# thygate/stable-diffusion-webui-depthmap-script

Hardware: AMD Instinct MI355X
Metric: depth+stereo pairs/sec @1024x1024 (higher is better)
Workload: dtype f16 (network) / f64 (stereo, normal map); 1 GPU; BASELINE config c3: MiDaS 3.1 DPT BEiT-L/16 512 forward (fp16, random-init weights seed 0, net 512x512, 1025 tokens) + depth->u16 + create_stereoimages(polylines_sharp, left-right, divergence 2.5%) + create_normalmap (Sobel 3) on 32 x 1024x1024 RGB per GPU, inputs resident in HBM; depth_network=dpt_beit_large_512, height=1024, width=1024, forward_launch=eager, library_convolutions=MIOpen, heuristic solver choice, overlap=single stream, parallelism=units sharded over 1 GPU(s), no data-path collective

## Files before the change

include/depthstereo.h:

```cpp
#ifndef DEPTHSTEREO_H
#define DEPTHSTEREO_H

#include <stddef.h>
#include <stdint.h>

#ifdef __cplusplus
extern "C" {
#endif

#define DS_VERSION 100

#define DS_OK            0
#define DS_EINVAL       -1
#define DS_EUNSUPPORTED -2
#define DS_EHIP         -3
#define DS_ENOMEM       -4

#define DS_DEPTH_U16 0
#define DS_DEPTH_F32 1
#define DS_DEPTH_F64 2

#define DS_FILL_NONE                0
#define DS_FILL_NAIVE               1
#define DS_FILL_NAIVE_INTERPOLATING 2
#define DS_FILL_POLYLINES_SOFT      3
#define DS_FILL_POLYLINES_SHARP     4

typedef struct ds_ctx ds_ctx;

int ds_version(void);
const char *ds_last_error(void);
int ds_ctx_create(ds_ctx **out, int device);
int ds_ctx_destroy(ds_ctx *ctx);

typedef struct ds_eye {
    double divergence_px;
    double separation_px;
    uint8_t *out;
    int64_t out_row_stride;
    int64_t out_img_stride;
} ds_eye;

int ds_stereo_warp(ds_ctx *ctx, const uint8_t *image, const void *depth, int depth_dtype,
                   int n, int h, int w, int c, double exponent, const double *pow_lut,
                   int fill, const ds_eye *eyes, int n_eyes, void *stream);

int ds_depth_minmax(ds_ctx *ctx, const void *depth, int depth_dtype, int n, int h, int w,
                    double *minmax_out, void *stream);

int ds_profile_enable(ds_ctx *ctx, int enable);
int ds_profile_last_ms(ds_ctx *ctx, float *render_ms, float *exact_ms);

#define DS_KT_LINEAR_GELU      0
#define DS_KT_ATTENTION        1
#define DS_KT_LINEAR_RESIDUAL  2
#define DS_KT_LINEAR           3
#define DS_KT_LINEAR_VT        4
#define DS_KT_CONV3X3          5
#define DS_KT_LINEAR_READOUT   6
#define DS_KT_LINEAR_SHUFFLE   7
#define DS_KT_NORMALMAP        8
#define DS_KT_RAGGED          12
int ds_kernel_timer_enable(ds_ctx *ctx, int enable);
int ds_kernel_timer_read(ds_ctx *ctx, int kind, int64_t *launches, double *total_ms);
int ds_kernel_timer_read_each(ds_ctx *ctx, int kind, float *ms_out, int64_t capacity, int64_t *launches);

int ds_stereo_last_exact_rows(ds_ctx *ctx, int64_t *rows_out, void *stream);
int ds_stereo_last_stats(ds_ctx *ctx, int64_t *stats_out, void *stream);

int ds_copy_view(ds_ctx *ctx, const uint8_t *src, int64_t src_row_stride, int64_t src_img_stride,
                 uint8_t *dst, int64_t dst_row_stride, int64_t dst_img_stride,
                 int n, int h, int64_t row_bytes, void *stream);

int ds_overlap_red_cyan(ds_ctx *ctx, const uint8_t *im1, int64_t im1_row_stride, int64_t im1_img_stride,
                        const uint8_t *im2, int64_t im2_row_stride, int64_t im2_img_stride,
                        int n, int h, int w, int c, uint8_t *out, void *stream);

int ds_normalmap(ds_ctx *ctx, const uint16_t *depth, int n, int h, int w, int pre_blur,
                 int sobel_ksize, int post_blur, int invert, uint8_t *out, void *stream);

int ds_normalmap_f64(ds_ctx *ctx, const double *depth, int n, int h, int w, int pre_blur,
                     int sobel_ksize, int post_blur, int invert, uint8_t *out, void *stream);

int ds_normalmap_gradient_f32(ds_ctx *ctx, const float *depth, int n, int h, int w, int invert, uint8_t *out, void *stream);

int ds_normalmap_gradient_f16(ds_ctx *ctx, const void *depth, int n, int h, int w, int invert, uint8_t *out, void *stream);

int ds_normalmap_gradient_blur_f32(ds_ctx *ctx, const float *depth, int n, int h, int w, int pre_blur, int post_blur, int invert,
                                   uint8_t *out, void *stream);

int ds_normalmap_wrap(ds_ctx *ctx, const uint16_t *depth, int n, int h, int w, int pre_blur,
                      int sobel_ksize, int post_blur, int invert, uint8_t *out, void *stream);
int ds_normalmap_f64_wrap(ds_ctx *ctx, const double *depth, int n, int h, int w, int pre_blur,
                          int sobel_ksize, int post_blur, int invert, uint8_t *out, void *stream);
int ds_normalmap_gradient_f32_wrap(ds_ctx *ctx, const float *depth, int n, int h, int w, int invert, uint8_t *out, void *stream);
int ds_normalmap_gradient_f16_wrap(ds_ctx *ctx, const void *depth, int n, int h, int w, int invert, uint8_t *out, void *stream);
int ds_normalmap_gradient_blur_f32_wrap(ds_ctx *ctx, const float *depth, int n, int h, int w, int pre_blur, int post_blur, int invert,
                                        uint8_t *out, void *stream);

int ds_bilateral_u16(ds_ctx *ctx, const uint16_t *depth, int n, int h, int w, int radius, const double *ws, const double *wr,
                     int wrap, double *out, void *stream);

int ds_normalmap_selfcheck(ds_ctx *ctx, unsigned long long k0, unsigned long long stride, unsigned long long count,
                           unsigned long long *mismatches, void *stream);

int ds_depth_to_u16(ds_ctx *ctx, const float *pred, int n, int h, int w, int invert,
                    uint16_t *out, float *norm_out, void *stream);

int ds_colorize_u16(ds_ctx *ctx, const uint16_t *depth, int n, int h, int w, const double *vmin_vmax,
                    const uint8_t *lut_rgba, int lut_n, uint8_t *out, void *stream);

int ds_convert_to_i16(ds_ctx *ctx, const void *arr, int is_f64, int64_t count, uint16_t *out, void *stream);

#define DS_PIX_U8  0
#define DS_PIX_U16 1
#define DS_PIX_I32 2
#define DS_PIX_F32 3

int ds_resize_lanczos(ds_ctx *ctx, const void *src, int pix, int n, int in_h, int in_w, int64_t src_px_stride, int64_t src_row_stride,
                      int64_t src_img_stride, void *dst, int out_h, int out_w, const int32_t *h_bounds, const void *h_coeffs, int h_taps,
                      const int32_t *v_bounds, const void *v_coeffs, int v_taps, void *tmp, void *stream);

#define DS_CD_WIDEN       0
#define DS_CD_SINGLE_BAND 1
#define DS_CD_MULTI_BAND  2
#define DS_CD_WORKSPACE_BLOCKS 256
int ds_custom_depth_to_f64(ds_ctx *ctx, const void *src, int pix, int n, int h, int w, int64_t src_px_stride, int64_t src_row_stride,
                           int64_t src_img_stride, int rule, double *out, double *workspace, void *stream);

#define DS_DTYPE_F16  1
#define DS_DTYPE_BF16 2
#define DS_DTYPE_F32  3

int ds_attention_fwd(ds_ctx *ctx, const void *qk, const void *vt, const void *bias_packed, void *out,
                     int B, int Np, int H, int n_valid, float scale, int dtype, void *stream);

int ds_attention_bias_pack(ds_ctx *ctx, const float *bias, int H, int n, int Np, int dtype, void *packed, void *stream);

int ds_attention_reload_env(void);

int ds_preprocess_bicubic(ds_ctx *ctx, const void *images, void *out, int batch, int in_h, int in_w, int out_h, int out_w,
                          int flip_channels, const float *mean, const float *std, int dtype, void *stream);

int ds_residual_layernorm(ds_ctx *ctx, const void *x, const void *branch, const void *gamma, const void *ln_weight,
                          const void *ln_bias, void *x_out, void *h_out, int64_t rows, int channels, float eps, int dtype,
                          void *stream);

int ds_reassemble_readout(ds_ctx *ctx, const void *proj, const void *clsvec, void *out, int batch, int tokens, int channels,
                          int dtype, void *stream);

int ds_bias_act_nhwc(ds_ctx *ctx, const void *x, const void *bias, const void *res1, const void *res2, void *out,
                     int64_t elements, int channels, int relu, int dtype, void *stream);

int ds_group_norm_nchw(ds_ctx *ctx, const void *x, const void *gamma, const void *beta, const void *res, void *out, int n, int channels,
                       int hw, int groups, float eps, int relu, int dtype, void *stream);

int ds_linear(ds_ctx *ctx, const void *x, const void *w, const void *bias, void *y, int64_t rows, int64_t out_features,
              int64_t in_features, int64_t ldy, int act, int dtype, void *stream);

int ds_linear_residual(ds_ctx *ctx, const void *x, const void *w, const void *bias, const void *gamma, const void *res, void *y,
                       int64_t rows, int64_t out_features, int64_t in_features, int dtype, void *stream);

int ds_linear_vt(ds_ctx *ctx, const void *w_v, const void *h, void *vt, int64_t channels, int64_t batch, int64_t tokens,
                 int64_t in_features, int dtype, void *stream);

int ds_linear_qkv(ds_ctx *ctx, const void *h, const void *w_qk, const void *b_qk, const void *w_v, void *qk, void *vt,
                  int64_t batch, int64_t tokens, int64_t qk_features, int64_t v_channels, int64_t in_features, int dtype, void *stream);

int ds_linear_shuffle(ds_ctx *ctx, const void *x, const void *w, const void *bias, void *y, int64_t pixels, int64_t in_features,
                      int width, int stride, int out_channels, int dtype, void *stream);

int ds_linear_readout(ds_ctx *ctx, const void *x, const void *w_tok, const void *cls_vec, void *y, int64_t images,
                      int64_t tokens_padded, int64_t tokens, int64_t out_features, int64_t in_features, int dtype, void *stream);

int ds_row_stats(ds_ctx *ctx, const void *x, void *stats, int64_t rows, int channels, float eps, int dtype, void *stream);
int ds_linear_ln(ds_ctx *ctx, const void *x, const void *w_scaled, const float *colsum, const void *bias, const void *stats, void *y,
                 int64_t rows, int64_t out_features, int64_t in_features, int64_t ldy, int act, int dtype, void *stream);
int ds_linear_vt_ln(ds_ctx *ctx, const void *w_v_scaled, const float *colsum, const void *x, const void *stats, void *vt,
                    int64_t channels, int64_t batch, int64_t tokens, int64_t in_features, int dtype, void *stream);

int ds_linear_reload_env(void);

int ds_conv3x3_nhwc(ds_ctx *ctx, const void *x, const void *w, const void *bias, const void *res1, const void *res2, void *y,
                    int batch, int height, int width, int in_channels, int out_channels, int act, int dtype, void *stream);

int ds_conv3x3_nhwc_circular(ds_ctx *ctx, const void *x, const void *w, const void *bias, const void *res1, const void *res2, void *y,
                             int batch, int height, int width, int in_channels, int out_channels, int act, int dtype, void *stream);

int ds_upsample_bilinear_nhwc(ds_ctx *ctx, const void *in, void *out, int batch, int channels, int in_h, int in_w,
                              int out_h, int out_w, int align_corners, int dtype, void *stream);

int ds_dpt_head_tail(ds_ctx *ctx, const void *x, int batch, int in_h, int in_w, int out_h, int out_w,
                     const void *conv3_wfrag, const float *conv3_bias, const float *conv1_weight, float conv1_bias,
                     int relu_out, void *out, int dtype, void *stream);

int ds_dpt_head_tail_circular(ds_ctx *ctx, const void *x, int batch, int in_h, int in_w, int out_h, int out_w,
                              const void *conv3_wfrag, const float *conv3_bias, const float *conv1_weight, float conv1_bias,
                              int relu_out, void *out, int dtype, void *stream);

int ds_gconv3x3_nhwc_f32(ds_ctx *ctx, const float *x, const float *w_gtio, const float *bias, float *y, int batch, int height, int width,
                         int channels, int channels_per_group, int relu, void *stream);
int ds_add_relu_f32(ds_ctx *ctx, const float *a, const float *b, float *y, int64_t count, void *stream);

int ds_bias_act_f32(ds_ctx *ctx, const float *x, const float *bias, const float *res, float *y, int64_t pixels, int channels, int relu,
                    void *stream);

int ds_dwconv_nhwc(ds_ctx *ctx, const void *x, const float *w, const float *bias_in, const float *bias, void *y, int batch, int in_h,
                   int in_w, int channels, int out_h, int out_w, int kernel, int stride, int pad_top, int pad_left, int dtype, void *stream);
int ds_relu_cat_f32(ds_ctx *ctx, const float *a, const float *b, float *y, int batch, int64_t plane, int channels_a, int channels_b, int layout,
                    void *stream);

int ds_boost_blend(ds_ctx *ctx, float *dst, int64_t dst_row_stride, int height, int width, const void *patches,
                   int n_patches, const float *preds, int pred_size, const float *mask_template, int mask_size,
                   void *stream);

#ifdef __cplusplus
}
#endif
#endif
```

stable-diffusion-webui-depthmap-script_amd/build_native.py:

```python
import os
import shutil
import subprocess
import sys

HERE = os.path.dirname(os.path.abspath(__file__))
CSRC = os.path.join(HERE, "csrc")
EXPERIMENTS = bool(os.environ.get("DS_EXPERIMENTS"))
OUT = os.path.join(HERE, "libdepthstereo_hip_experiments.so" if EXPERIMENTS else "libdepthstereo_hip.so")
OBJ_DIR = os.path.join(HERE, "build", "experiments") if EXPERIMENTS else os.path.join(HERE, "build")
SOURCES = ["ds_api.hip", "ds_stereo.hip", "ds_stereo_polylines.hip", "ds_normalmap.hip", "ds_attention.hip", "ds_attention4.hip", "ds_encoder_ops.hip", "ds_boost.hip", "ds_heatmap.hip", "ds_linear.hip", "ds_gconv.hip", "ds_dwconv.hip", "ds_resample.hip", "ds_bilateral.hip"]
FLAGS = ["--offload-arch=gfx950", "-O3", "-std=c++17", "-ffp-contract=off", "-fno-fast-math", "-fPIC",
         "-fvisibility=hidden", "-Wall", "-Wno-unused-function",
         "-mllvm", "-amdgpu-mfma-vgpr-form=1"]


if EXPERIMENTS:
    FLAGS.append("-DDS_EXPERIMENTS")


EXTRA_FLAGS = {"ds_attention4.hip": ["-fno-slp-vectorize"]}


def hipcc():
    for cand in (shutil.which("hipcc"), "/opt/rocm/bin/hipcc"):
        if cand and os.path.exists(cand):
            return cand
    raise RuntimeError("hipcc not found")


def needs_build():
    if not os.path.exists(OUT):
        return True
    t = os.path.getmtime(OUT)
    deps = [os.path.join(CSRC, f) for f in os.listdir(CSRC)] + [os.path.join(HERE, "..", "include", "depthstereo.h")]
    return any(os.path.getmtime(d) > t for d in deps)


def build(force=False, verbose=True):
    if not force and not needs_build():
        return OUT
    objs = []
    procs = []
    os.makedirs(OBJ_DIR, exist_ok=True)
    for s in SOURCES:
        o = os.path.join(OBJ_DIR, s.replace(".hip", ".o"))
        cmd = [hipcc()] + FLAGS + EXTRA_FLAGS.get(s, []) + ["-c", os.path.join(CSRC, s), "-o", o]
        if verbose:
            print(" ".join(cmd), flush=True)
        procs.append((s, subprocess.Popen(cmd)))
        objs.append(o)
    for s, p in procs:
        if p.wait() != 0:
            raise RuntimeError(f"hipcc failed on {s}")
    cmd = [hipcc(), "--offload-arch=gfx950", "-shared", "-fPIC", "-o", OUT] + objs
    if verbose:
        print(" ".join(cmd), flush=True)
    subprocess.check_call(cmd)
    return OUT


if __name__ == "__main__":
    build(force="--force" in sys.argv)
    print(OUT)
```

stable-diffusion-webui-depthmap-script_amd/csrc/ds_common.h:

```cpp
#pragma once
#include <hip/hip_runtime.h>
#include <stdint.h>
#include <stdio.h>
#include <string.h>

#include "../../include/depthstereo.h"

#define DS_API extern "C" __attribute__((visibility("default")))

void ds_set_error(const char *fmt, ...);

#define DS_HIP_CHECK(expr)                                                              \
    do {                                                                                \
        hipError_t _e = (expr);                                                         \
        if (_e != hipSuccess) {                                                         \
            ds_set_error("%s failed: %s (%s:%d)", #expr, hipGetErrorString(_e), __FILE__, __LINE__); \
            return DS_EHIP;                                                             \
        }                                                                               \
    } while (0)

#define DS_REQUIRE(cond, code, ...)      \
    do {                                 \
        if (!(cond)) {                   \
            ds_set_error(__VA_ARGS__);   \
            return (code);               \
        }                                \
    } while (0)

#define DS_KT_KINDS 24
#define DS_KT_RING 1024
struct ds_ctx {
    int device;
    void *minmax;      size_t minmax_bytes;
    void *partials;    size_t partials_bytes;
    void *row_flags;   size_t row_flags_bytes;
    void *row_list;    size_t row_list_bytes;
    void *exact_ws;    size_t exact_ws_bytes;
    void *tmp_a;       size_t tmp_a_bytes;
    void *tmp_b;       size_t tmp_b_bytes;
    void *zero_line;   size_t zero_line_bytes;
    int zero_line_cleared;
    void *lin_ws;      size_t lin_ws_bytes;
    void *lin_ws_cleared;
    void *gn_ws;       size_t gn_ws_bytes;
    int ncu;
    int64_t last_exact_rows_valid;
    int profile;
    hipEvent_t ev[4];
    int ev_created, ev_recorded;
    int ktimer;
    hipEvent_t (*kt_ev[DS_KT_KINDS])[2];
    int kt_n[DS_KT_KINDS];
};

int ds_kt_begin(ds_ctx *ctx, int kind, hipStream_t st);
void ds_kt_end(ds_ctx *ctx, int kind, int slot, hipStream_t st);

int ds_ctx_reserve(ds_ctx *ctx, void **slot, size_t *cur, size_t need);

__device__ __forceinline__ uint8_t ds_f64_to_u8(double v)
{
    if (!(v == v)) return 0;
    if (v >= 9.2e18 || v <= -9.2e18) return 0;
    return (uint8_t)(long long)v;
}

__device__ __forceinline__ int ds_reflect101(int i, int n)
{
    if (n == 1) return 0;
    while (i < 0 || i >= n) { if (i < 0) i = -i; else i = 2 * (n - 1) - i; }
    return i;
}
__device__ __forceinline__ int ds_mod(int i, int n)
{
    i %= n;
    return i < 0 ? i + n : i;
}
__device__ __forceinline__ int ds_wrap_prev(int i, int n) { return i > 0 ? i - 1 : n - 1; }
__device__ __forceinline__ int ds_wrap_next(int i, int n) { return i + 1 < n ? i + 1 : 0; }

__device__ __forceinline__ double ds_wave_min(double v)
{
    for (int o = 32; o > 0; o >>= 1) { double t = __shfl_xor(v, o, 64); v = t < v ? t : v; }
    return v;
}
__device__ __forceinline__ double ds_wave_max(double v)
{
    for (int o = 32; o > 0; o >>= 1) { double t = __shfl_xor(v, o, 64); v = t > v ? t : v; }
    return v;
}

template <int DT> struct ds_depth_traits;
template <> struct ds_depth_traits<DS_DEPTH_U16> {
    typedef uint16_t T;
    __device__ static __forceinline__ double norm(T v, double mn, double mx) {
        return (double)(uint16_t)(v - (uint16_t)mn) / (double)(uint16_t)((uint16_t)mx - (uint16_t)mn);
    }
};
template <> struct ds_depth_traits<DS_DEPTH_F32> {
    typedef float T;
    __device__ static __forceinline__ double norm(T v, double mn, double mx) {
        float den = (float)mx - (float)mn;
        float q = (v - (float)mn) / den;
        return (double)q;
    }
};
template <> struct ds_depth_traits<DS_DEPTH_F64> {
    typedef double T;
    __device__ static __forceinline__ double norm(T v, double mn, double mx) {
        return (v - mn) / (mx - mn);
    }
};
```

stable-diffusion-webui-depthmap-script_amd/csrc/ds_encoder_ops.hip:

```cpp
#include <stdlib.h>
#include <string.h>

#include <algorithm>

#include "ds_common.h"

template <int BF16> struct eo_traits;
template <> struct eo_traits<0> { typedef _Float16 T; };
template <> struct eo_traits<1> { typedef __bf16 T; };

template <int BF16, int EPL, int W>
__global__ __launch_bounds__(256) void k_residual_layernorm(const void *x_, const void *o_, const void *gamma_, const void *lnw_,
                                                             const void *lnb_, void *xout_, void *hout_, int M, float eps)
{
    typedef typename eo_traits<BF16>::T T;
    constexpr int C = EPL * 64;
    const int lane = threadIdx.x & 63;
    const int row = blockIdx.x * 4 + (threadIdx.x >> 6);
    if (row >= M) return;
    const T *x = (const T *)x_ + (size_t)row * C;
    const T *o = o_ ? (const T *)o_ + (size_t)row * C : nullptr;
    const T *gamma = (const T *)gamma_, *lnw = (const T *)lnw_, *lnb = (const T *)lnb_;
    T *xout = xout_ ? (T *)xout_ + (size_t)row * C : nullptr;
    T *hout = (T *)hout_ + (size_t)row * C;
    float v[EPL];
    float sum = 0.f;
#pragma unroll
    for (int k = 0; k < EPL / W; k++) {
        const int idx = (k * 64 + lane) * W;
        T xv[W], ov[W], gv[W];
        __builtin_memcpy(xv, x + idx, sizeof(xv));
        if (o) {
            __builtin_memcpy(ov, o + idx, sizeof(ov));
            if (gamma) __builtin_memcpy(gv, gamma + idx, sizeof(gv));
        }
        T rv[W];
#pragma unroll
        for (int t = 0; t < W; t++) {
            float f = (float)xv[t];
            if (o) f += (gamma ? (float)gv[t] : 1.0f) * (float)ov[t];
            rv[t] = (T)f;
            v[k * W + t] = (float)rv[t];
            sum += v[k * W + t];
        }
        if (o && xout) __builtin_memcpy(xout + idx, rv, sizeof(rv));
    }
#pragma unroll
    for (int s = 32; s > 0; s >>= 1) sum += __shfl_xor(sum, s, 64);
    const float mean = sum * (1.0f / C);
    float sq = 0.f;
#pragma unroll
    for (int i = 0; i < EPL; i++) { const float d = v[i] - mean; sq += d * d; }
#pragma unroll
    for (int s = 32; s > 0; s >>= 1) sq += __shfl_xor(sq, s, 64);
    const float rstd = rsqrtf(sq * (1.0f / C) + eps);
#pragma unroll
    for (int k = 0; k < EPL / W; k++) {
        const int idx = (k * 64 + lane) * W;
        T wv[W], bv[W], hv[W];
        __builtin_memcpy(wv, lnw + idx, sizeof(wv));
        __builtin_memcpy(bv, lnb + idx, sizeof(bv));
#pragma unroll
        for (int t = 0; t < W; t++) hv[t] = (T)((v[k * W + t] - mean) * rstd * (float)wv[t] + (float)bv[t]);
        __builtin_memcpy(hout + idx, hv, sizeof(hv));
    }
}

template <int BF16>
static int eo_launch(int C, const void *x, const void *o, const void *gamma, const void *lnw, const void *lnb, void *xout, void *hout,
                     int M, float eps, hipStream_t st)
{
    dim3 grid((M + 3) / 4), block(256);
    switch (C) {
    case 384: hipLaunchKernelGGL((k_residual_layernorm<BF16, 6, 2>), grid, block, 0, st, x, o, gamma, lnw, lnb, xout, hout, M, eps); break;
    case 768: hipLaunchKernelGGL((k_residual_layernorm<BF16, 12, 4>), grid, block, 0, st, x, o, gamma, lnw, lnb, xout, hout, M, eps); break;
    case 1024: hipLaunchKernelGGL((k_residual_layernorm<BF16, 16, 8>), grid, block, 0, st, x, o, gamma, lnw, lnb, xout, hout, M, eps); break;
    case 1536: hipLaunchKernelGGL((k_residual_layernorm<BF16, 24, 8>), grid, block, 0, st, x, o, gamma, lnw, lnb, xout, hout, M, eps); break;
    default: ds_set_error("ds_residual_layernorm: channel count %d not built (384, 768, 1024, 1536)", C); return DS_EUNSUPPORTED;
    }
    return DS_OK;
}

DS_API int ds_residual_layernorm(ds_ctx *ctx, const void *x, const void *branch, const void *gamma, const void *ln_weight,
                                 const void *ln_bias, void *x_out, void *h_out, int64_t rows, int channels, float eps, int dtype,
                                 void *stream)
{
    DS_REQUIRE(ctx && x && ln_weight && ln_bias && h_out, DS_EINVAL, "ds_residual_layernorm: null argument");
    DS_REQUIRE(rows > 0 && rows < (1ll << 31), DS_EINVAL, "ds_residual_layernorm: bad row count");
    DS_REQUIRE(dtype == DS_DTYPE_F16 || dtype == DS_DTYPE_BF16, DS_EINVAL, "ds_residual_layernorm: dtype must be f16 or bf16");
    DS_REQUIRE(branch == nullptr || x_out != nullptr, DS_EINVAL, "ds_residual_layernorm: x_out is required with a branch");
    DS_REQUIRE(((uintptr_t)x & 15) == 0 && ((uintptr_t)h_out & 15) == 0 && ((uintptr_t)branch & 15) == 0 && ((uintptr_t)x_out & 15) == 0,
               DS_EINVAL, "ds_residual_layernorm: operands must be 16-byte aligned");
    DS_HIP_CHECK(hipSetDevice(ctx->device));
    int rc = dtype == DS_DTYPE_F16
        ? eo_launch<0>(channels, x, branch, gamma, ln_weight, ln_bias, x_out, h_out, (int)rows, eps, (hipStream_t)stream)
        : eo_launch<1>(channels, x, branch, gamma, ln_weight, ln_bias, x_out, h_out, (int)rows, eps, (hipStream_t)stream);
    if (rc) return rc;
    DS_HIP_CHECK(hipGetLastError());
    return DS_OK;
}

template <int BF16, int EPL, int W>
__global__ __launch_bounds__(256) void k_row_stats(const void *x_, float2 *stats, int M, float eps)
{
    typedef typename eo_traits<BF16>::T T;
    constexpr int C = EPL * 64;
    const int lane = threadIdx.x & 63;
    const int row = blockIdx.x * 4 + (threadIdx.x >> 6);
    if (row >= M) return;
    const T *x = (const T *)x_ + (size_t)row * C;
    float v[EPL];
    float sum = 0.f;
#pragma unroll
    for (int k = 0; k < EPL / W; k++) {
        T xv[W];
        __builtin_memcpy(xv, x + (k * 64 + lane) * W, sizeof(xv));
#pragma unroll
        for (int t = 0; t < W; t++) { v[k * W + t] = (float)xv[t]; sum += v[k * W + t]; }
    }
#pragma unroll
    for (int s = 32; s > 0; s >>= 1) sum += __shfl_xor(sum, s, 64);
    const float mean = sum * (1.0f / C);
    float sq = 0.f;
#pragma unroll
    for (int i = 0; i < EPL; i++) { const float d = v[i] - mean; sq += d * d; }
#pragma unroll
    for (int s = 32; s > 0; s >>= 1) sq += __shfl_xor(sq, s, 64);
    const float rstd = rsqrtf(sq * (1.0f / C) + eps);
    if (lane == 0) stats[row] = make_float2(rstd, -mean * rstd);
}

DS_API int ds_row_stats(ds_ctx *ctx, const void *x, void *stats, int64_t rows, int channels, float eps, int dtype, void *stream)
{
    DS_REQUIRE(ctx && x && stats, DS_EINVAL, "ds_row_stats: null argument");
    DS_REQUIRE(rows > 0 && rows < (1ll << 31), DS_EINVAL, "ds_row_stats: bad row count");
    DS_REQUIRE(dtype == DS_DTYPE_F16 || dtype == DS_DTYPE_BF16, DS_EINVAL, "ds_row_stats: dtype must be f16 or bf16");
    DS_REQUIRE(((uintptr_t)x & 15) == 0 && ((uintptr_t)stats & 15) == 0, DS_EINVAL, "ds_row_stats: operands must be 16-byte aligned");
    DS_HIP_CHECK(hipSetDevice(ctx->device));
    dim3 grid((unsigned)((rows + 3) / 4)), block(256);
    hipStream_t st = (hipStream_t)stream;
    float2 *out = (float2 *)stats;
    const int M = (int)rows;
#define RS_CASE(C_, EPL_, W_) case C_: if (dtype == DS_DTYPE_F16) hipLaunchKernelGGL((k_row_stats<0, EPL_, W_>), grid, block, 0, st, x, out, M, eps); \
                                       else hipLaunchKernelGGL((k_row_stats<1, EPL_, W_>), grid, block, 0, st, x, out, M, eps); break;
    switch (channels) {
    RS_CASE(384, 6, 2) RS_CASE(768, 12, 4) RS_CASE(1024, 16, 8) RS_CASE(1536, 24, 8)
    default: ds_set_error("ds_row_stats: channel count %d not built (384, 768, 1024, 1536)", channels); return DS_EUNSUPPORTED;
    }
#undef RS_CASE
    DS_HIP_CHECK(hipGetLastError());
    return DS_OK;
}

template <int BF16>
__global__ __launch_bounds__(256) void k_upsample_bilinear_nhwc(const void *in_, void *out_, int C8, int ih, int iw, int oh, int ow,
                                                                 float sy, float sx, int align_corners)
{
    typedef typename eo_traits<BF16>::T T;
    const unsigned i = blockIdx.x * 256u + threadIdx.x;
    if (i >= (unsigned)ow * (unsigned)C8) return;
    const int ox = (int)(i / (unsigned)C8), c8 = (int)(i - (unsigned)ox * (unsigned)C8);
    const int b = blockIdx.z;
    float fx;
    if (align_corners) fx = sx * ox;
    else fx = fmaxf(sx * (ox + 0.5f) - 0.5f, 0.f);
    const int x0 = min((int)fx, iw - 1), x1 = min(x0 + 1, iw - 1);
    const float tx = fx - x0;
    const T *in = (const T *)in_ + (size_t)b * ih * iw * C8 * 8 + (size_t)c8 * 8;
    int py0 = -1, py1 = -1;
    T a[8], bq[8], c[8], d[8], o[8];
#pragma unroll
    for (int r = 0; r < 2; r++) {
        const int oy = 2 * (int)blockIdx.y + r;
        if (oy >= oh) break;
        float fy;
        if (align_corners) fy = sy * oy;
        else fy = fmaxf(sy * (oy + 0.5f) - 0.5f, 0.f);
        const int y0 = min((int)fy, ih - 1), y1 = min(y0 + 1, ih - 1);
        const float ty = fy - y0;
        if (y0 == py1 && y0 != py0) {
#pragma unroll
            for (int k = 0; k < 8; k++) { a[k] = c[k]; bq[k] = d[k]; }
        } else if (y0 != py0) {
            __builtin_memcpy(a, in + ((size_t)y0 * iw + x0) * C8 * 8, 16);
            __builtin_memcpy(bq, in + ((size_t)y0 * iw + x1) * C8 * 8, 16);
        }
        if (y1 != py1 || r == 0) {
            if (y1 == y0) {
#pragma unroll
                for (int k = 0; k < 8; k++) { c[k] = a[k]; d[k] = bq[k]; }
            } else {
                __builtin_memcpy(c, in + ((size_t)y1 * iw + x0) * C8 * 8, 16);
                __builtin_memcpy(d, in + ((size_t)y1 * iw + x1) * C8 * 8, 16);
            }
        }
        py0 = y0; py1 = y1;
        const float w00 = (1.f - ty) * (1.f - tx), w01 = (1.f - ty) * tx, w10 = ty * (1.f - tx), w11 = ty * tx;
#pragma unroll
        for (int k = 0; k < 8; k++)
            o[k] = (T)(w00 * (float)a[k] + w01 * (float)bq[k] + w10 * (float)c[k] + w11 * (float)d[k]);
        __builtin_memcpy((T *)out_ + ((((size_t)b * oh + oy) * ow) * C8 + i) * 8, o, 16);
    }
}

DS_API int ds_upsample_bilinear_nhwc(ds_ctx *ctx, const void *in, void *out, int batch, int channels, int in_h, int in_w,
                                     int out_h, int out_w, int align_corners, int dtype, void *stream)
{
    DS_REQUIRE(ctx && in && out, DS_EINVAL, "ds_upsample_bilinear_nhwc: null argument");
    DS_REQUIRE(batch > 0 && channels > 0 && (channels % 8) == 0 && in_h > 0 && in_w > 0 && out_h > 0 && out_w > 0, DS_EINVAL,
               "ds_upsample_bilinear_nhwc: bad shape (channels must be a multiple of 8)");
    DS_REQUIRE(dtype == DS_DTYPE_F16 || dtype == DS_DTYPE_BF16, DS_EINVAL, "ds_upsample_bilinear_nhwc: dtype must be f16 or bf16");
    DS_REQUIRE(((uintptr_t)in & 15) == 0 && ((uintptr_t)out & 15) == 0, DS_EINVAL, "ds_upsample_bilinear_nhwc: 16-byte alignment");
    DS_HIP_CHECK(hipSetDevice(ctx->device));
    float sy, sx;
    if (align_corners) {
        sy = out_h > 1 ? (float)(in_h - 1) / (float)(out_h - 1) : 0.f;
        sx = out_w > 1 ? (float)(in_w - 1) / (float)(out_w - 1) : 0.f;
    } else {
        sy = (float)in_h / (float)out_h;
        sx = (float)in_w / (float)out_w;
    }
    const int C8 = channels / 8;
    DS_REQUIRE((long long)out_w * C8 < (1ll << 31) && out_h <= 65535 && batch <= 65535, DS_EUNSUPPORTED, "ds_upsample_bilinear_nhwc: tensor too large");
    dim3 grid((unsigned)(((long long)out_w * C8 + 255) / 256), (unsigned)((out_h + 1) / 2), (unsigned)batch);
    if (dtype == DS_DTYPE_F16)
        hipLaunchKernelGGL((k_upsample_bilinear_nhwc<0>), grid, dim3(256), 0, (hipStream_t)stream, in, out, C8, in_h, in_w, out_h, out_w, sy, sx, align_corners);
    else
        hipLaunchKernelGGL((k_upsample_bilinear_nhwc<1>), grid, dim3(256), 0, (hipStream_t)stream, in, out, C8, in_h, in_w, out_h, out_w, sy, sx, align_corners);
    DS_HIP_CHECK(hipGetLastError());
    return DS_OK;
}

struct PreParams {
    const uint8_t *in;
    void *out;
    int B, ih, iw, oh, ow, flip;
    float sy, sx;
    float mean[3], istd[3];
    long long total;
};

__device__ __forceinline__ void pre_cubic(float t, float *c)
{
    const float A = -0.75f;
    const float x0 = t + 1.0f, x3 = 2.0f - t, x2 = 1.0f - t;
    c[0] = ((A * x0 - 5.0f * A) * x0 + 8.0f * A) * x0 - 4.0f * A;
    c[1] = ((A + 2.0f) * t - (A + 3.0f)) * t * t + 1.0f;
    c[2] = ((A + 2.0f) * x2 - (A + 3.0f)) * x2 * x2 + 1.0f;
    c[3] = ((A * x3 - 5.0f * A) * x3 + 8.0f * A) * x3 - 4.0f * A;
}

template <int DT>
__global__ __launch_bounds__(256) void k_preprocess_bicubic(PreParams P)
{
    const long long idx = (long long)blockIdx.x * 256 + threadIdx.x;
    if (idx >= P.total) return;
    const int ox = (int)(idx % P.ow);
    long long r = idx / P.ow;
    const int oy = (int)(r % P.oh);
    const int b = (int)(r / P.oh);
    const float fy = P.sy * ((float)oy + 0.5f) - 0.5f, fx = P.sx * ((float)ox + 0.5f) - 0.5f;
    const float fy0 = floorf(fy), fx0 = floorf(fx);
    float cy[4], cx[4];
    pre_cubic(fy - fy0, cy);
    pre_cubic(fx - fx0, cx);
    const int iy = (int)fy0, ix = (int)fx0;
    const uint8_t *img = P.in + (size_t)b * P.ih * P.iw * 3;
    float acc[3] = {0.f, 0.f, 0.f};
#pragma unroll
    for (int ky = 0; ky < 4; ky++) {
        const int y = min(max(iy - 1 + ky, 0), P.ih - 1);
        const uint8_t *row = img + (size_t)y * P.iw * 3;
        float h[3] = {0.f, 0.f, 0.f};
#pragma unroll
        for (int kx = 0; kx < 4; kx++) {
            const int x = min(max(ix - 1 + kx, 0), P.iw - 1);
            const uint8_t *px = row + (size_t)x * 3;
#pragma unroll
            for (int c = 0; c < 3; c++) h[c] += cx[kx] * ((float)px[c] / 255.0f);
        }
#pragma unroll
        for (int c = 0; c < 3; c++) acc[c] += cy[ky] * h[c];
    }
    float o[3];
#pragma unroll
    for (int c = 0; c < 3; c++) o[c] = (acc[P.flip ? 2 - c : c] - P.mean[c]) * P.istd[c];
    if (DT == 2) {
        float *q = (float *)P.out + (size_t)idx * 3;
        q[0] = o[0]; q[1] = o[1]; q[2] = o[2];
    } else {
        typedef typename eo_traits<DT == 1 ? 1 : 0>::T T;
        T *q = (T *)P.out + (size_t)idx * 3;
        q[0] = (T)o[0]; q[1] = (T)o[1]; q[2] = (T)o[2];
    }
}

DS_API int ds_preprocess_bicubic(ds_ctx *ctx, const void *images, void *out, int batch, int in_h, int in_w, int out_h, int out_w,
                                 int flip_channels, const float *mean, const float *std, int dtype, void *stream)
{
    DS_REQUIRE(ctx && images && out && mean && std, DS_EINVAL, "ds_preprocess_bicubic: null argument");
    DS_REQUIRE(batch > 0 && in_h > 0 && in_w > 0 && out_h > 0 && out_w > 0, DS_EINVAL, "ds_preprocess_bicubic: bad shape");
    DS_REQUIRE(dtype == DS_DTYPE_F16 || dtype == DS_DTYPE_BF16 || dtype == DS_DTYPE_F32, DS_EINVAL, "ds_preprocess_bicubic: dtype must be f16, bf16 or f32");
    DS_REQUIRE(std[0] != 0.f && std[1] != 0.f && std[2] != 0.f, DS_EINVAL, "ds_preprocess_bicubic: std must be non-zero");
    DS_HIP_CHECK(hipSetDevice(ctx->device));
    PreParams P;
    P.in = (const uint8_t *)images; P.out = out;
    P.B = batch; P.ih = in_h; P.iw = in_w; P.oh = out_h; P.ow = out_w; P.flip = flip_channels ? 1 : 0;
    P.sy = (float)in_h / (float)out_h; P.sx = (float)in_w / (float)out_w;
    for (int c = 0; c < 3; c++) { P.mean[c] = mean[c]; P.istd[c] = 1.0f / std[c]; }
    P.total = (long long)batch * out_h * out_w;
    DS_REQUIRE((P.total + 255) / 256 < (1ll << 31), DS_EUNSUPPORTED, "ds_preprocess_bicubic: tensor too large");
    dim3 grid((unsigned)((P.total + 255) / 256));
    hipStream_t st = (hipStream_t)stream;
    if (dtype == DS_DTYPE_F16) hipLaunchKernelGGL((k_preprocess_bicubic<0>), grid, dim3(256), 0, st, P);
    else if (dtype == DS_DTYPE_BF16) hipLaunchKernelGGL((k_preprocess_bicubic<1>), grid, dim3(256), 0, st, P);
    else hipLaunchKernelGGL((k_preprocess_bicubic<2>), grid, dim3(256), 0, st, P);
    DS_HIP_CHECK(hipGetLastError());
    return DS_OK;
}

#define HT_TW 32
#define HT_PW (HT_TW + 2)

typedef _Float16 ht_f16x8 __attribute__((ext_vector_type(8)));
typedef __bf16 ht_bf16x8 __attribute__((ext_vector_type(8)));
typedef float ht_f32x16 __attribute__((ext_vector_type(16)));

struct HeadTailParams {
    const void *x;
    const void *wfrag;
    const float *b2, *w3;
    void *out;
    float b3;
    int B, ih, iw, oh, ow, relu_out;
    float sy, sx;
};

template <int BF16, int RPW, int CIRC = 0>
__global__ __launch_bounds__(256) void k_dpt_head_tail(HeadTailParams P)
{
    typedef typename eo_traits<BF16>::T T;
    constexpr int HT_TH = 4 * RPW;
    constexpr int HT_NPIX = (HT_TH + 2) * HT_PW;
    extern __shared__ __attribute__((aligned(16))) unsigned char s_act[];
    const int tid = threadIdx.x, wave = tid >> 6, lane = tid & 63, hi = lane >> 5, l31 = lane & 31;
    const int b = blockIdx.z, ty0 = blockIdx.y * HT_TH, tx0 = blockIdx.x * HT_TW;
    const T *x = (const T *)P.x + (size_t)b * P.ih * P.iw * 128;

    for (int i0 = tid; i0 < HT_NPIX * 16; i0 += 256 * 4) {
        T a[4][8], bq[4][8], cq[4][8], d[4][8];
        float w00[4], w01[4], w10[4], w11[4];
        bool inside[4], live[4];
#pragma unroll
        for (int u = 0; u < 4; u++) {
            const int i = i0 + u * 256;
            live[u] = i < HT_NPIX * 16;
            const int pix = min(i, HT_NPIX * 16 - 1) >> 4, chunk = i & 15;
            const int r = pix / HT_PW, c = pix - r * HT_PW;
            int oy = ty0 - 1 + r, ox = tx0 - 1 + c;
            if constexpr (CIRC) {
                oy = oy < 0 ? oy + P.oh : (oy >= P.oh ? oy - P.oh : oy);
                ox = ox < 0 ? ox + P.ow : (ox >= P.ow ? ox - P.ow : ox);
                oy = min(oy, P.oh - 1); ox = min(ox, P.ow - 1);
                inside[u] = live[u];
            } else {
                inside[u] = live[u] && oy >= 0 && oy < P.oh && ox >= 0 && ox < P.ow;
            }
            const float fy = P.sy * max(oy, 0), fx = P.sx * max(ox, 0);
            const int y0 = min((int)fy, P.ih - 1), x0 = min((int)fx, P.iw - 1);
            const int y1 = min(y0 + 1, P.ih - 1), x1 = min(x0 + 1, P.iw - 1);
            const float ty = fy - y0, tx = fx - x0;
            w00[u] = (1.f - ty) * (1.f - tx); w01[u] = (1.f - ty) * tx; w10[u] = ty * (1.f - tx); w11[u] = ty * tx;
            __builtin_memcpy(a[u], x + ((size_t)y0 * P.iw + x0) * 128 + chunk * 8, 16);
            __builtin_memcpy(bq[u], x + ((size_t)y0 * P.iw + x1) * 128 + chunk * 8, 16);
            __builtin_memcpy(cq[u], x + ((size_t)y1 * P.iw + x0) * 128 + chunk * 8, 16);
            __builtin_memcpy(d[u], x + ((size_t)y1 * P.iw + x1) * 128 + chunk * 8, 16);
        }
#pragma unroll
        for (int u = 0; u < 4; u++) {
            if (!live[u]) continue;
            const int i = i0 + u * 256;
            const int pix = i >> 4, chunk = i & 15;
            T o[8];
#pragma unroll
            for (int k = 0; k < 8; k++)
                o[k] = inside[u] ? (T)(w00[u] * (float)a[u][k] + w01[u] * (float)bq[u][k] + w10[u] * (float)cq[u][k] + w11[u] * (float)d[u][k])
                                 : (T)0.f;
            __builtin_memcpy(s_act + pix * 256 + ((chunk ^ (pix & 15)) << 4), o, 16);
        }
    }
    __syncthreads();

    ht_f32x16 acc[RPW];
#pragma unroll
    for (int rr = 0; rr < RPW; rr++)
#pragma unroll
        for (int r = 0; r < 16; r++) acc[rr][r] = 0.f;
    const T *wf = (const T *)P.wfrag + ((size_t)hi * 32 + l31) * 8;
#pragma unroll
    for (int tap = 0; tap < 9; tap++) {
        const int dy = tap / 3, dx = tap - dy * 3;
#pragma unroll
        for (int s = 0; s < 8; s++) {
            uint4 wraw = *reinterpret_cast<const uint4 *>(wf + (size_t)(tap * 8 + s) * 2 * 32 * 8);
#pragma unroll
            for (int rr = 0; rr < RPW; rr++) {
                const int pix = (RPW * wave + rr + dy) * HT_PW + l31 + dx;
                const uint4 araw = *reinterpret_cast<const uint4 *>(s_act + pix * 256 + (((2 * s + hi) ^ (pix & 15)) << 4));
                if (BF16) {
                    union { uint4 u; ht_bf16x8 v; } wa, ab; wa.u = wraw; ab.u = araw;
                    acc[rr] = __builtin_amdgcn_mfma_f32_32x32x16_bf16(wa.v, ab.v, acc[rr], 0, 0, 0);
                } else {
                    union { uint4 u; ht_f16x8 v; } wa, ab; wa.u = wraw; ab.u = araw;
                    acc[rr] = __builtin_amdgcn_mfma_f32_32x32x16_f16(wa.v, ab.v, acc[rr], 0, 0, 0);
                }
            }
        }
    }
#pragma unroll
    for (int rr = 0; rr < RPW; rr++) {
        float part = 0.f;
#pragma unroll
        for (int r = 0; r < 16; r++) {
            const int ch = (r & 3) + 8 * (r >> 2) + 4 * hi;
            const float v = fmaxf(acc[rr][r] + P.b2[ch], 0.f);
            part += P.w3[ch] * v;
        }
        part += __shfl_xor(part, 32, 64);
        float res = part + P.b3;
        if (P.relu_out) res = fmaxf(res, 0.f);
        const int oy = ty0 + RPW * wave + rr, ox = tx0 + l31;
        if (hi == 0 && oy < P.oh && ox < P.ow) ((T *)P.out)[((size_t)b * P.oh + oy) * P.ow + ox] = (T)res;
    }
}

#define HTP_TH 8
#define HTP_NPIX ((HTP_TH + 2) * HT_PW)
#define HTP_W_BYTES (9 * 8 * 2 * 32 * 8 * 2)

template <int BF16>
__global__ __launch_bounds__(512) void k_dpt_head_tail_p(HeadTailParams P, int tiles_x, int tiles_y, int ntiles, int chunk)
{
    typedef typename eo_traits<BF16>::T T;
    extern __shared__ __attribute__((aligned(16))) unsigned char s_all[];
    unsigned char *s_w = s_all, *s_act = s_all + HTP_W_BYTES;
    const int tid = threadIdx.x, wave = tid >> 6, lane = tid & 63, hi = lane >> 5, l31 = lane & 31;
    for (int i = tid; i < HTP_W_BYTES / 16; i += 512)
        reinterpret_cast<uint4 *>(s_w)[i] = reinterpret_cast<const uint4 *>(P.wfrag)[i];
    for (int orig = blockIdx.x; orig < 8 * chunk; orig += gridDim.x) {
        const int tile = (orig & 7) * chunk + (orig >> 3);
        if (tile >= ntiles) continue;
        const int txi = tile % tiles_x, tyi = (tile / tiles_x) % tiles_y, b = tile / (tiles_x * tiles_y);
        const int ty0 = tyi * HTP_TH, tx0 = txi * HT_TW;
        const T *x = (const T *)P.x + (size_t)b * P.ih * P.iw * 128;
        __syncthreads();
        for (int i0 = tid; i0 < HTP_NPIX * 16; i0 += 512 * 4) {
            T a[4][8], bq[4][8], cq[4][8], d[4][8];
            float w00[4], w01[4], w10[4], w11[4];
            bool inside[4], live[4];
#pragma unroll
            for (int u = 0; u < 4; u++) {
                const int i = i0 + u * 512;
                live[u] = i < HTP_NPIX * 16;
                const int pix = min(i, HTP_NPIX * 16 - 1) >> 4, chunk16 = i & 15;
                const int r = pix / HT_PW, c = pix - r * HT_PW;
                const int oy = ty0 - 1 + r, ox = tx0 - 1 + c;
                inside[u] = live[u] && oy >= 0 && oy < P.oh && ox >= 0 && ox < P.ow;
                const float fy = P.sy * max(oy, 0), fx = P.sx * max(ox, 0);
                const int y0 = min((int)fy, P.ih - 1), x0 = min((int)fx, P.iw - 1);
                const int y1 = min(y0 + 1, P.ih - 1), x1 = min(x0 + 1, P.iw - 1);
                const float ty = fy - y0, tx = fx - x0;
                w00[u] = (1.f - ty) * (1.f - tx); w01[u] = (1.f - ty) * tx; w10[u] = ty * (1.f - tx); w11[u] = ty * tx;
                __builtin_memcpy(a[u], x + ((size_t)y0 * P.iw + x0) * 128 + chunk16 * 8, 16);
                __builtin_memcpy(bq[u], x + ((size_t)y0 * P.iw + x1) * 128 + chunk16 * 8, 16);
                __builtin_memcpy(cq[u], x + ((size_t)y1 * P.iw + x0) * 128 + chunk16 * 8, 16);
                __builtin_memcpy(d[u], x + ((size_t)y1 * P.iw + x1) * 128 + chunk16 * 8, 16);
            }
#pragma unroll
            for (int u = 0; u < 4; u++) {
                if (!live[u]) continue;
                const int i = i0 + u * 512;
                const int pix = i >> 4, chunk16 = i & 15;
                T o[8];
#pragma unroll
                for (int k = 0; k < 8; k++)
                    o[k] = inside[u] ? (T)(w00[u] * (float)a[u][k] + w01[u] * (float)bq[u][k] + w10[u] * (float)cq[u][k] + w11[u] * (float)d[u][k])
                                     : (T)0.f;
                __builtin_memcpy(s_act + pix * 256 + ((chunk16 ^ (pix & 15)) << 4), o, 16);
            }
        }
        __syncthreads();
        ht_f32x16 acc;
#pragma unroll
        for (int r = 0; r < 16; r++) acc[r] = 0.f;
        const unsigned char *wf = s_w + ((size_t)hi * 32 + l31) * 16;
#pragma unroll
        for (int tap = 0; tap < 9; tap++) {
            const int dy = tap / 3, dx = tap - dy * 3;
            const int pix = (wave + dy) * HT_PW + l31 + dx;
#pragma unroll
            for (int s8 = 0; s8 < 8; s8++) {
                const uint4 wraw = *reinterpret_cast<const uint4 *>(wf + (size_t)(tap * 8 + s8) * 2 * 32 * 16);
                const uint4 araw = *reinterpret_cast<const uint4 *>(s_act + pix * 256 + (((2 * s8 + hi) ^ (pix & 15)) << 4));
                if (BF16) {
                    union { uint4 u; ht_bf16x8 v; } wa, ab; wa.u = wraw; ab.u = araw;
                    acc = __builtin_amdgcn_mfma_f32_32x32x16_bf16(wa.v, ab.v, acc, 0, 0, 0);
                } else {
                    union { uint4 u; ht_f16x8 v; } wa, ab; wa.u = wraw; ab.u = araw;
                    acc = __builtin_amdgcn_mfma_f32_32x32x16_f16(wa.v, ab.v, acc, 0, 0, 0);
                }
            }
        }
        float part = 0.f;
#pragma unroll
        for (int r = 0; r < 16; r++) {
            const int ch = (r & 3) + 8 * (r >> 2) + 4 * hi;
            const float v = fmaxf(acc[r] + P.b2[ch], 0.f);
            part += P.w3[ch] * v;
        }
        part += __shfl_xor(part, 32, 64);
        float res = part + P.b3;
        if (P.relu_out) res = fmaxf(res, 0.f);
        const int oy = ty0 + wave, ox = tx0 + l31;
        if (hi == 0 && oy < P.oh && ox < P.ow) ((T *)P.out)[((size_t)b * P.oh + oy) * P.ow + ox] = (T)res;
    }
}

#define HTS_RING 10
#define HTS_PIXB 272
#define HTS_ROWB (HT_PW * HTS_PIXB)
#define HTS_ACT_BYTES (HTS_RING * HTS_ROWB)
#define HTS_PART_BYTES (4 * 4 * 64 * 16)
#define HTS_SRC_ROWS 4
#define HTS_SRC_COLS 7
#define HTS_SRC_LOADS (HTS_SRC_ROWS * HTS_SRC_COLS * 16 / 64)
#define HTS_STAGE_BYTES (HTS_SRC_ROWS * HTS_SRC_COLS * 256)
#define HTS_LDS_BYTES (HTS_ACT_BYTES + 2 * HTS_PART_BYTES + 256 + 4 * HTS_STAGE_BYTES)
#define HTS_NIT 9

__device__ __forceinline__ void hts_barrier()
{
    asm volatile("s_waitcnt lgkmcnt(0)" ::: "memory");
    __builtin_amdgcn_s_barrier();
    asm volatile("" ::: "memory");
}

struct HtsCols {
    int cx0[HTS_NIT], cx1[HTS_NIT];
    float wx0[HTS_NIT], wx1[HTS_NIT];
    int xlo;
};

template <int BF16>
// ... 656 lines not shown
```

stable-diffusion-webui-depthmap-script_amd/dmidas/backbones/beit.py:

```python
import torch
import torch.nn as nn
import torch.nn.functional as F

from src import vit_mi355x as vm


def gen_relative_position_index(window_size):
    num_relative_distance = (2 * window_size[0] - 1) * (2 * window_size[1] - 1) + 3
    window_area = window_size[0] * window_size[1]
    coords = torch.stack(torch.meshgrid([torch.arange(window_size[0]), torch.arange(window_size[1])], indexing='ij'))
    coords_flatten = torch.flatten(coords, 1)
    relative_coords = coords_flatten[:, :, None] - coords_flatten[:, None, :]
    relative_coords = relative_coords.permute(1, 2, 0).contiguous()
    relative_coords[:, :, 0] += window_size[0] - 1
    relative_coords[:, :, 1] += window_size[1] - 1
    relative_coords[:, :, 0] *= 2 * window_size[1] - 1
    relative_position_index = torch.zeros(size=(window_area + 1,) * 2, dtype=relative_coords.dtype)
    relative_position_index[1:, 1:] = relative_coords.sum(-1)
    relative_position_index[0, 0:] = num_relative_distance - 3
    relative_position_index[0:, 0] = num_relative_distance - 2
    relative_position_index[0, 0] = num_relative_distance - 1
    return relative_position_index


class _Attention(nn.Module):

    def __init__(self, dim, num_heads, window_size):
        super().__init__()
        self.qkv = nn.Linear(dim, dim * 3, bias=False)
        self.q_bias = nn.Parameter(torch.zeros(dim))
        self.v_bias = nn.Parameter(torch.zeros(dim))
        self.window_size = window_size
        self.num_relative_distance = (2 * window_size[0] - 1) * (2 * window_size[1] - 1) + 3
        self.relative_position_bias_table = nn.Parameter(torch.zeros(self.num_relative_distance, num_heads))
        self.proj = nn.Linear(dim, dim)


class Block(vm.EncoderBlock):

    def __init__(self, dim, num_heads, window_size, mlp_ratio=4.0, init_values=1e-5):
        super().__init__(dim, num_heads, mlp_ratio)
        self.norm1 = nn.LayerNorm(dim, eps=1e-6)
        self.attn = _Attention(dim, num_heads, window_size)
        self.norm2 = nn.LayerNorm(dim, eps=1e-6)
        self.mlp = vm.Mlp(dim, int(dim * mlp_ratio))
        self.gamma_1 = nn.Parameter(init_values * torch.ones(dim))
        self.gamma_2 = nn.Parameter(init_values * torch.ones(dim))
        self._bias_cache = {}

    def qkv_weights(self):
        c = self.dim
        w = self.attn.qkv.weight
        qb = self.attn.q_bias
        key = (qb._version, qb.data_ptr(), qb.dtype)
        hit = getattr(self, "_bqk", None)
        if hit is None or hit[0] != key:
            if hit is not None:
                vm.cache_evicted()
            b_qk = torch.cat((qb, torch.zeros_like(qb)))
            hit = (key, b_qk)
            if not torch.is_grad_enabled():
                self._bqk = hit
        return w[:2 * c], hit[1], w[2 * c:], self.attn.v_bias

    def proj(self, o, b_v=None):
        return vm.linear(o, self.attn.proj.weight, vm.folded_proj_bias(self.attn.proj, b_v))

    def gammas(self):
        return self.gamma_1, self.gamma_2

    def _resized_table(self, window_size):
        a = self.attn
        old_h, old_w = 2 * a.window_size[0] - 1, 2 * a.window_size[1] - 1
        new_h, new_w = 2 * window_size[0] - 1, 2 * window_size[1] - 1
        table = a.relative_position_bias_table
        old_sub = table[:a.num_relative_distance - 3].reshape(1, old_w, old_h, -1).permute(0, 3, 1, 2)
        new_sub = F.interpolate(old_sub.float(), size=(int(new_h), int(new_w)), mode="bilinear").to(table.dtype)
        new_sub = new_sub.permute(0, 2, 3, 1).reshape(new_h * new_w, -1)
        return torch.cat([new_sub, table[a.num_relative_distance - 3:]])

    def rel_pos_bias(self, window_size):
        new_table = self._resized_table(window_size)
        index = _relative_position_index(tuple(window_size), new_table.device)
        n = window_size[0] * window_size[1] + 1
        bias = new_table[index.view(-1)].view(n, n, -1)
        return bias.permute(2, 0, 1).contiguous()

    def attention_bias(self, n_pad, grid_hw, dtype, device):
        a = self.attn
        plain = dtype in (torch.float32, torch.float64) or device.type != 'cuda' or vm.STOCK[0]
        if not plain:
            n_pad = (n_pad + 63) // 64 * 64
        key = (tuple(grid_hw), n_pad, dtype, device, a.relative_position_bias_table._version, plain)
        hit = self._bias_cache.get(key)
        if hit is not None:
            return hit
        with torch.no_grad():
            if plain:
                heads = a.relative_position_bias_table.shape[1]
                if heads * n_pad * n_pad * 4 > DENSE_BIAS_BYTES_MAX:
                    if self._bias_cache:
                        self._bias_cache.clear()
                        vm.cache_evicted()
                    return _LazyBias(self._resized_table(tuple(grid_hw)).to(device=device, dtype=dtype), tuple(grid_hw), n_pad)
                bias = self.rel_pos_bias(tuple(grid_hw))
                n = bias.shape[-1]
                bt = torch.zeros((bias.shape[0], n_pad, n_pad), dtype=dtype, device=device)
                bt[:, :n, :n] = bias
            else:
                from src import _native
                bt = _native.attention_bias_pack(self.rel_pos_bias(tuple(grid_hw)).to(device), n_pad, dtype)
        return vm.cache_store(self._bias_cache, key, bt, entries=2)


DENSE_BIAS_BYTES_MAX = 256 << 20
_index_cache = {}


def _relative_position_index(window_size, device):
    key = (tuple(window_size), str(device))
    hit = _index_cache.get(key)
    if hit is None:
        hit = vm.cache_store(_index_cache, key, gen_relative_position_index(window_size).to(device))
    return hit


class _LazyBias:

    def __init__(self, table, window_size, n_pad):
        self.table, self.window_size, self.n_pad = table, window_size, n_pad
        self.n = window_size[0] * window_size[1] + 1

    def rows(self, q0, q1):
        index = _relative_position_index(self.window_size, self.table.device)
        out = self.table.new_zeros((self.table.shape[1], q1 - q0, self.n_pad))
        qe = min(q1, self.n)
        if qe > q0:
            out[:, :qe - q0, :self.n] = self.table[index[q0:qe].reshape(-1)].view(qe - q0, self.n, -1).permute(2, 0, 1)
        return out


class PatchEmbed(nn.Module):
    def __init__(self, patch_size, embed_dim):
        super().__init__()
        self.proj = nn.Conv2d(3, embed_dim, kernel_size=patch_size, stride=patch_size)

    def forward(self, x):
        if vm.patch_embed_hip_ok(self.proj, x):
            return vm.patch_embed_tokens(self.proj, x)
        return self.proj(x).flatten(2).transpose(1, 2)


class Beit(nn.Module):

    def __init__(self, img_size, embed_dim, depth, num_heads, init_values, num_classes=1000):
        super().__init__()
        self.patch_size = [16, 16]
        self.embed_dim = embed_dim
        window = (img_size // 16, img_size // 16)
        self.patch_embed = PatchEmbed(16, embed_dim)
        self.cls_token = nn.Parameter(torch.zeros(1, 1, embed_dim))
        self.blocks = nn.ModuleList([Block(embed_dim, num_heads, window, 4.0, init_values) for _ in range(depth)])
        self.fc_norm = nn.LayerNorm(embed_dim, eps=1e-6)
        self.head = nn.Linear(embed_dim, num_classes)
        nn.init.trunc_normal_(self.cls_token, std=0.02)
        for m in self.modules():
            if isinstance(m, nn.Linear):
                nn.init.trunc_normal_(m.weight, std=0.02)
                if m.bias is not None:
                    nn.init.zeros_(m.bias)

    def forward_taps(self, x, hooks, padded=False):
        grid = (x.shape[2] // 16, x.shape[3] // 16)
        t = self.patch_embed(x)
        t = torch.cat((self.cls_token.expand(t.shape[0], -1, -1).to(t.dtype), t), dim=1)
        n_valid = t.shape[1]
        t = vm.pad_tokens(t, vm.pad_len(n_valid, t.shape[0]))
        _, taps = vm.run_blocks(self.blocks, t, n_valid, grid, set(hooks), padded_taps=padded)
        return [taps[i] for i in hooks], grid, n_valid


class ProjectReadout(nn.Module):

    def __init__(self, in_features, start_index=1):
        super().__init__()
        self.start_index = start_index
        self.project = nn.Sequential(nn.Linear(2 * in_features, in_features), nn.GELU())

    def _split(self):
        lin = self.project[0]
        key = (lin.weight._version, lin.weight.data_ptr(), lin.weight.dtype)
        hit = getattr(self, "_w_split", None)
        if hit is None or hit[0] != key:
            if hit is not None:
                vm.cache_evicted()
            c = lin.in_features // 2
            hit = (key, lin.weight[:, :c].contiguous(), lin.weight[:, c:].contiguous())
            if not torch.is_grad_enabled():
                self._w_split = hit
        return hit[1], hit[2]

    def forward(self, x):
        if self.start_index != 1:
            readout = x[:, 0].unsqueeze(1).expand_as(x[:, self.start_index:])
            return self.project(torch.cat((x[:, self.start_index:], readout), -1))
        w_tok, w_cls = self._split()
        clsvec = F.linear(x[:, 0], w_cls, self.project[0].bias)
        proj = F.linear(x, w_tok)
        if vm.half_on_gpu(x) and x.shape[-1] % 8 == 0:
            from src import _native
            return _native.reassemble_readout(proj, clsvec)
        return F.gelu(proj[:, 1:] + clsvec[:, None])

    def forward_padded(self, xp, n_valid):
        from src import _native
        w_tok, w_cls = self._split()
        if (self.start_index == 1 and vm.READOUT_HIP and vm.LINEAR_HIP == "all" and vm.half_on_gpu(xp) and xp.is_contiguous()
                and _native.linear_readout_supported(xp, w_tok) and vm.hip_gemm_ok(xp.shape[0] * xp.shape[1], w_tok.shape[0])):
            x0 = xp[:, 0].contiguous()
            if vm.invariant() and _native.linear_supported(x0, w_cls):
                clsvec = _native.linear(x0, w_cls, self.project[0].bias)
            else:
                clsvec = F.linear(x0, w_cls, self.project[0].bias)
            return _native.linear_readout(xp, n_valid, w_tok, clsvec)
        return self.forward(xp[:, :n_valid])


class _Skip(nn.Module):
    def forward(self, x):
        return x


def _postprocess(vit_features, out_features, tail):
    return nn.Sequential(ProjectReadout(vit_features), _Skip(), _Skip(), nn.Conv2d(vit_features, out_features, 1), *tail)


class BeitBackbone(nn.Module):

    def __init__(self, model, features, vit_features, hooks):
        super().__init__()
        self.model = model
        self.hooks = list(hooks)
        f = features
        self.act_postprocess1 = _postprocess(vit_features, f[0], [nn.ConvTranspose2d(f[0], f[0], 4, 4, 0)])
        self.act_postprocess2 = _postprocess(vit_features, f[1], [nn.ConvTranspose2d(f[1], f[1], 2, 2, 0)])
        self.act_postprocess3 = _postprocess(vit_features, f[2], [])
        self.act_postprocess4 = _postprocess(vit_features, f[3], [nn.Conv2d(f[3], f[3], 3, 2, 1)])

    def forward(self, x):
        taps, grid, n_valid = self.model.forward_taps(x, self.hooks, padded=True)
        outs = []
        for tap, post in zip(taps, (self.act_postprocess1, self.act_postprocess2, self.act_postprocess3, self.act_postprocess4)):
            y = post[0].forward_padded(tap, n_valid)
            y = y.reshape(y.shape[0], grid[0], grid[1], y.shape[2]).permute(0, 3, 1, 2)
            for layer in list(post)[3:]:
                y = vm.conv_module(layer, y)
            outs.append(y)
        return outs


def make_beit(name, hooks):
    cfg = {"beitl16_512": (512, 1024, 24, 16, [256, 512, 1024, 1024]),
           "beitl16_384": (384, 1024, 24, 16, [256, 512, 1024, 1024]),
           "beitb16_384": (384, 768, 12, 12, [96, 192, 384, 768])}[name]
    img, dim, depth, heads, features = cfg
    model = Beit(img, dim, depth, heads, init_values=1e-5 if dim == 1024 else 0.1)
    return BeitBackbone(model, features, dim, hooks), features
```

stable-diffusion-webui-depthmap-script_amd/dmidas/dpt_depth.py:

```python
import numpy as np
import torch
import torch.nn as nn
import torch.nn.functional as F

from src import vit_mi355x as vm

from .backbones.beit import make_beit
from .backbones.vit import make_vit

_HOOKS = {"beitl16_512": [5, 11, 17, 23], "beitl16_384": [5, 11, 17, 23], "beitb16_384": [2, 5, 8, 11],
          "vitl16_384": [5, 11, 17, 23], "vitb_rn50_384": [0, 1, 8, 11]}


class ResidualConvUnit_custom(nn.Module):
    def __init__(self, features):
        super().__init__()
        self.conv1 = nn.Conv2d(features, features, kernel_size=3, stride=1, padding=1, bias=True)
        self.conv2 = nn.Conv2d(features, features, kernel_size=3, stride=1, padding=1, bias=True)

    def forward(self, x):
        return vm.residual_conv_unit(self.conv1, self.conv2, x)


class FeatureFusionBlock_custom(nn.Module):
    def __init__(self, features):
        super().__init__()
        self.out_conv = nn.Conv2d(features, features, kernel_size=1, stride=1, padding=0, bias=True)
        self.resConfUnit1 = ResidualConvUnit_custom(features)
        self.resConfUnit2 = ResidualConvUnit_custom(features)

    def forward(self, *xs, size=None):
        output = xs[0]
        if len(xs) == 2:
            output = vm.residual_conv_unit(self.resConfUnit1.conv1, self.resConfUnit1.conv2, xs[1], skip=output)
        output = self.resConfUnit2(output)
        output = vm.conv_module(self.out_conv, output)
        if size is None:
            return vm.interpolate_bilinear(output, scale_factor=2, align_corners=True)
        return vm.interpolate_bilinear(output, size=tuple(size), align_corners=True)


class Interpolate(nn.Module):
    def __init__(self, scale_factor, mode, align_corners=False):
        super().__init__()
        self.scale_factor, self.mode, self.align_corners = scale_factor, mode, align_corners

    def forward(self, x):
        if self.mode == "bilinear":
            return vm.interpolate_bilinear(x, scale_factor=self.scale_factor, align_corners=bool(self.align_corners))
        return F.interpolate(x, scale_factor=self.scale_factor, mode=self.mode, align_corners=self.align_corners)


class DPT(nn.Module):
    def __init__(self, head, features=256, backbone="beitl16_512", readout="project", channels_last=False, use_bn=False, **kwargs):
        super().__init__()
        if backbone not in _HOOKS:
            raise NotImplementedError(f"DPT backbone '{backbone}' is not built (built: {sorted(_HOOKS)})")
        if readout != "project" or use_bn:
            raise NotImplementedError("only readout='project', use_bn=False (what src/depthmap_generation.py:129-176 uses)")
        self.channels_last = channels_last
        self.size_routed = backbone == "vitb_rn50_384"
        make = make_beit if backbone.startswith("beit") else make_vit
        self.pretrained, in_shape = make(backbone, _HOOKS[backbone])
        scratch = nn.Module()
        for i in range(4):
            setattr(scratch, f"layer{i + 1}_rn", nn.Conv2d(in_shape[i], features, kernel_size=3, stride=1, padding=1, bias=False))
        for i in range(1, 5):
            setattr(scratch, f"refinenet{i}", FeatureFusionBlock_custom(features))
        scratch.output_conv = head
        self.scratch = scratch

    def forward(self, x, features=None):
        if getattr(self, "size_routed", False):
            with vm.size_routed():
                return self._forward(x, features)
        return self._forward(x, features)

    def _forward(self, x, features=None):
        l1, l2, l3, l4 = self.pretrained(x)
        s = self.scratch
        l1, l2, l3, l4 = vm.conv2d(s.layer1_rn, l1), vm.conv2d(s.layer2_rn, l2), vm.conv2d(s.layer3_rn, l3), vm.conv2d(s.layer4_rn, l4)
        path_4 = s.refinenet4(l4, size=l3.shape[2:])
        path_3 = s.refinenet3(path_4, l3, size=l2.shape[2:])
        path_2 = s.refinenet2(path_3, l2, size=l1.shape[2:])
        path_1 = s.refinenet1(path_2, l1)
        head = s.output_conv
        if features is not None:
            features.update(l4_rn=l4, r4=path_4, r3=path_3, r2=path_2, r1=path_1)
            y = path_1
            for i, layer in enumerate(head):
                y = layer(y)
                if i == 3:
                    features['out_conv'] = y
            return y
        if (vm.half_on_gpu(path_1) and isinstance(head[1], Interpolate)
                and head[1].mode == "bilinear" and head[1].align_corners and tuple(head[2].weight.shape) == (32, 128, 3, 3)
                and head[2].padding_mode in ('zeros', 'circular') and vm.circular_hip_ok(head[2])):
            from src import _native
            y = vm.conv2d(head[0], path_1) if vm.conv3x3_hip_ok(head[0], path_1) else vm.conv_module(head[0], path_1)
            size = (int(y.shape[2] * head[1].scale_factor), int(y.shape[3] * head[1].scale_factor))
            return _native.dpt_head_tail(y, size, head[2], head[4], relu_out=isinstance(head[5], nn.ReLU))
        return head(path_1)


def _constrain(x, multiple, min_val=0, max_val=None):
    y = int(np.round(x / multiple) * multiple)
    if max_val is not None and y > max_val:
        y = int(np.floor(x / multiple) * multiple)
    if y < min_val:
        y = int(np.ceil(x / multiple) * multiple)
    return y


def midas_net_size(width, height, net_w, net_h, resize_method="minimal", multiple=32):
    scale_h, scale_w = net_h / height, net_w / width
    if resize_method == "lower_bound":
        scale_h = scale_w = max(scale_w, scale_h)
    elif resize_method == "upper_bound":
        scale_h = scale_w = min(scale_w, scale_h)
    elif resize_method == "minimal":
        if abs(1 - scale_w) < abs(1 - scale_h):
            scale_h = scale_w
        else:
            scale_w = scale_h
    else:
        raise ValueError(f"resize_method {resize_method} not implemented")
    if resize_method == "lower_bound":
        return _constrain(scale_w * width, multiple, min_val=net_w), _constrain(scale_h * height, multiple, min_val=net_h)
    if resize_method == "upper_bound":
        return _constrain(scale_w * width, multiple, max_val=net_w), _constrain(scale_h * height, multiple, max_val=net_h)
    return _constrain(scale_w * width, multiple), _constrain(scale_h * height, multiple)


class DPTDepthModel(DPT):
    def __init__(self, path=None, non_negative=True, **kwargs):
        features = kwargs.get("features", 256)
        head_features_1 = kwargs.pop("head_features_1", features)
        head_features_2 = kwargs.pop("head_features_2", 32)
        head = nn.Sequential(
            nn.Conv2d(head_features_1, head_features_1 // 2, kernel_size=3, stride=1, padding=1),
            Interpolate(scale_factor=2, mode="bilinear", align_corners=True),
            nn.Conv2d(head_features_1 // 2, head_features_2, kernel_size=3, stride=1, padding=1),
            nn.ReLU(True),
            nn.Conv2d(head_features_2, 1, kernel_size=1, stride=1, padding=0),
            nn.ReLU(True) if non_negative else nn.Identity(),
            nn.Identity())
        super().__init__(head, **kwargs)
        if path is not None:
            self.load(path)

    def load(self, path):
        parameters = torch.load(path, map_location=torch.device('cpu'))
        if "optimizer" in parameters:
            parameters = parameters["model"]
        self.load_state_dict(parameters, strict=False)

    @vm.deterministic_forward
    def forward(self, x, features=None):
        return super().forward(x, features).squeeze(dim=1)

    @staticmethod
    def preprocess(images_u8, net_size=512, net_h=None, resize_mode="minimal", mean=0.5, std=0.5, dtype=None):
        b, h, w, _ = images_u8.shape
        nw, nh = midas_net_size(w, h, int(net_size), int(net_size if net_h is None else net_h), resize_mode)
        if images_u8.is_cuda and vm.PREPROCESS_HIP and not vm.STOCK[0]:
            from src import _native
            return _native.preprocess_bicubic(images_u8, (nh, nw), mean, std, flip=True, dtype=dtype)
        x = images_u8.flip(-1).permute(0, 3, 1, 2).float() / 255.0
        x = F.interpolate(x, size=(nh, nw), mode="bicubic", align_corners=False)
        if hasattr(mean, "__len__"):
            mean = vm.device_constant(mean, x.device).view(1, 3, 1, 1)
            std = vm.device_constant(std, x.device).view(1, 3, 1, 1)
        x = (x - mean) / std
        return x if dtype is None else x.to(dtype)

    @torch.no_grad()
    def infer_batch(self, images_u8, net_size=512, resize_mode="minimal", mean=0.5, std=0.5, net_h=None):
        b, h, w, _ = images_u8.shape
        dtype = self.scratch.layer1_rn.weight.dtype
        x = self.preprocess(images_u8, net_size, net_h, resize_mode, mean, std, dtype=dtype)
        if x.is_cuda:
            x = x.contiguous(memory_format=torch.channels_last)
        pred = self.forward(x)
        pred = F.interpolate(pred.unsqueeze(1), size=(h, w), mode="bicubic", align_corners=False).squeeze(1)
        return pred.float()
```

stable-diffusion-webui-depthmap-script_amd/src/_native.py:

```python
import collections
import ctypes
import math
import os
import threading

import numpy as np

_PKG_ROOT = os.path.dirname(os.path.dirname(os.path.abspath(__file__)))
LIB_PATH = os.environ.get("DS_NATIVE_LIB") or os.path.join(_PKG_ROOT, "libdepthstereo_hip.so")

DS_DEPTH_U16, DS_DEPTH_F32, DS_DEPTH_F64 = 0, 1, 2
FILL_IDS = {"none": 0, "naive": 1, "naive_interpolating": 2, "polylines_soft": 3, "polylines_sharp": 4}

EXPORTS = [
    "ds_version", "ds_last_error", "ds_normalmap_f64", "ds_normalmap_gradient_f32", "ds_reassemble_readout", "ds_bias_act_nhwc", "ds_linear", "ds_linear_residual", "ds_linear_vt", "ds_linear_qkv", "ds_conv3x3_nhwc", "ds_ctx_create", "ds_ctx_destroy", "ds_stereo_warp", "ds_depth_minmax",
    "ds_stereo_last_exact_rows", "ds_copy_view", "ds_overlap_red_cyan", "ds_normalmap", "ds_depth_to_u16",
    "ds_convert_to_i16", "ds_profile_enable", "ds_profile_last_ms", "ds_stereo_last_stats", "ds_attention_fwd", "ds_attention_bias_pack", "ds_colorize_u16", "ds_residual_layernorm", "ds_boost_blend", "ds_upsample_bilinear_nhwc", "ds_dpt_head_tail", "ds_preprocess_bicubic", "ds_linear_reload_env", "ds_attention_reload_env", "ds_normalmap_selfcheck", "ds_normalmap_gradient_f16", "ds_normalmap_gradient_blur_f32",
    "ds_linear_shuffle", "ds_linear_readout", "ds_kernel_timer_enable", "ds_kernel_timer_read", "ds_kernel_timer_read_each", "ds_group_norm_nchw",
    "ds_row_stats", "ds_linear_ln", "ds_linear_vt_ln", "ds_gconv3x3_nhwc_f32", "ds_add_relu_f32", "ds_bias_act_f32", "ds_relu_cat_f32",
    "ds_dwconv_nhwc", "ds_resize_lanczos", "ds_custom_depth_to_f64", "ds_conv3x3_nhwc_circular", "ds_dpt_head_tail_circular",
    "ds_normalmap_wrap", "ds_normalmap_f64_wrap", "ds_normalmap_gradient_f32_wrap", "ds_normalmap_gradient_f16_wrap", "ds_normalmap_gradient_blur_f32_wrap",
    "ds_bilateral_u16",
]


class DepthStereoError(RuntimeError):
    pass


class ds_eye(ctypes.Structure):
    _fields_ = [("divergence_px", ctypes.c_double), ("separation_px", ctypes.c_double),
                ("out", ctypes.c_void_p), ("out_row_stride", ctypes.c_int64), ("out_img_stride", ctypes.c_int64)]


_lib = None
_lib_lock = threading.Lock()

CALLS = collections.Counter()


def lib():
    global _lib
    with _lib_lock:
        if _lib is None:
            if not os.path.exists(LIB_PATH):
                raise DepthStereoError(
                    f"{LIB_PATH} is missing: build it with `python __graft_entry__.py build` "
                    "(hipcc --offload-arch=gfx950).  There is no CPU fallback.")
            L = ctypes.CDLL(LIB_PATH)
            vp, ci, cd, i64 = ctypes.c_void_p, ctypes.c_int, ctypes.c_double, ctypes.c_int64
            L.ds_version.restype = ci
            L.ds_last_error.restype = ctypes.c_char_p
            L.ds_ctx_create.argtypes = [ctypes.POINTER(vp), ci]
            L.ds_ctx_destroy.argtypes = [vp]
            L.ds_stereo_warp.argtypes = [vp, vp, vp, ci, ci, ci, ci, ci, cd, vp, ci, ctypes.POINTER(ds_eye), ci, vp]
            L.ds_depth_minmax.argtypes = [vp, vp, ci, ci, ci, ci, vp, vp]
            L.ds_stereo_last_exact_rows.argtypes = [vp, ctypes.POINTER(i64), vp]
            L.ds_copy_view.argtypes = [vp, vp, i64, i64, vp, i64, i64, ci, ci, i64, vp]
            L.ds_overlap_red_cyan.argtypes = [vp, vp, i64, i64, vp, i64, i64, ci, ci, ci, ci, vp, vp]
            L.ds_normalmap.argtypes = [vp, vp, ci, ci, ci, ci, ci, ci, ci, vp, vp]
            L.ds_normalmap_f64.argtypes = [vp, vp, ci, ci, ci, ci, ci, ci, ci, vp, vp]
            L.ds_normalmap_gradient_f32.argtypes = [vp, vp, ci, ci, ci, ci, vp, vp]
            L.ds_normalmap_gradient_f16.argtypes = [vp, vp, ci, ci, ci, ci, vp, vp]
            L.ds_normalmap_gradient_blur_f32.argtypes = [vp, vp, ci, ci, ci, ci, ci, ci, vp, vp]
            for name in ("ds_normalmap", "ds_normalmap_f64", "ds_normalmap_gradient_f32", "ds_normalmap_gradient_f16", "ds_normalmap_gradient_blur_f32"):
                getattr(L, name + "_wrap").argtypes = getattr(L, name).argtypes
            L.ds_bilateral_u16.argtypes = [vp, vp, ci, ci, ci, ci, vp, vp, ci, vp, vp]
            L.ds_depth_to_u16.argtypes = [vp, vp, ci, ci, ci, ci, vp, vp, vp]
            L.ds_convert_to_i16.argtypes = [vp, vp, ci, i64, vp, vp]
            L.ds_stereo_last_stats.argtypes = [vp, ctypes.POINTER(i64), vp]
            L.ds_attention_fwd.argtypes = [vp, vp, vp, vp, vp, ci, ci, ci, ci, ctypes.c_float, ci, vp]
            L.ds_normalmap_selfcheck.argtypes = [vp, ctypes.c_ulonglong, ctypes.c_ulonglong, ctypes.c_ulonglong, ctypes.POINTER(ctypes.c_ulonglong), vp]
            L.ds_attention_bias_pack.argtypes = [vp, vp, ci, ci, ci, ci, vp, vp]
            L.ds_colorize_u16.argtypes = [vp, vp, ci, ci, ci, vp, vp, ci, vp, vp]
            L.ds_residual_layernorm.argtypes = [vp, vp, vp, vp, vp, vp, vp, vp, i64, ci, ctypes.c_float, ci, vp]
            L.ds_boost_blend.argtypes = [vp, vp, i64, ci, ci, vp, ci, vp, ci, vp, ci, vp]
            L.ds_upsample_bilinear_nhwc.argtypes = [vp, vp, vp, ci, ci, ci, ci, ci, ci, ci, ci, vp]
            L.ds_dpt_head_tail.argtypes = [vp, vp, ci, ci, ci, ci, ci, vp, vp, vp, ctypes.c_float, ci, vp, ci, vp]
            L.ds_dpt_head_tail_circular.argtypes = L.ds_dpt_head_tail.argtypes
            L.ds_preprocess_bicubic.argtypes = [vp, vp, vp, ci, ci, ci, ci, ci, ci, ctypes.POINTER(ctypes.c_float),
                                                ctypes.POINTER(ctypes.c_float), ci, vp]
            L.ds_reassemble_readout.argtypes = [vp, vp, vp, vp, ci, ci, ci, ci, vp]
            L.ds_bias_act_nhwc.argtypes = [vp, vp, vp, vp, vp, vp, i64, ci, ci, ci, vp]
            L.ds_group_norm_nchw.argtypes = [vp, vp, vp, vp, vp, vp, ci, ci, ci, ci, ctypes.c_float, ci, ci, vp]
            L.ds_linear.argtypes = [vp, vp, vp, vp, vp, i64, i64, i64, i64, ci, ci, vp]
            L.ds_linear_residual.argtypes = [vp, vp, vp, vp, vp, vp, vp, i64, i64, i64, ci, vp]
            L.ds_linear_vt.argtypes = [vp, vp, vp, vp, i64, i64, i64, i64, ci, vp]
            L.ds_linear_qkv.argtypes = [vp, vp, vp, vp, vp, vp, vp, i64, i64, i64, i64, i64, ci, vp]
            L.ds_conv3x3_nhwc.argtypes = [vp, vp, vp, vp, vp, vp, vp, ci, ci, ci, ci, ci, ci, ci, vp]
            L.ds_conv3x3_nhwc_circular.argtypes = L.ds_conv3x3_nhwc.argtypes
            L.ds_linear_shuffle.argtypes = [vp, vp, vp, vp, vp, i64, i64, ci, ci, ci, ci, vp]
            L.ds_linear_readout.argtypes = [vp, vp, vp, vp, vp, i64, i64, i64, i64, i64, ci, vp]
            L.ds_row_stats.argtypes = [vp, vp, vp, i64, ci, ctypes.c_float, ci, vp]
            L.ds_linear_ln.argtypes = [vp, vp, vp, vp, vp, vp, vp, i64, i64, i64, i64, ci, ci, vp]
            L.ds_linear_vt_ln.argtypes = [vp, vp, vp, vp, vp, vp, i64, i64, i64, i64, ci, vp]
            L.ds_gconv3x3_nhwc_f32.argtypes = [vp, vp, vp, vp, vp, ci, ci, ci, ci, ci, ci, vp]
            L.ds_add_relu_f32.argtypes = [vp, vp, vp, vp, i64, vp]
            L.ds_bias_act_f32.argtypes = [vp, vp, vp, vp, vp, i64, ci, ci, vp]
            L.ds_relu_cat_f32.argtypes = [vp, vp, vp, vp, ci, i64, ci, ci, ci, vp]
            L.ds_dwconv_nhwc.argtypes = [vp, vp, vp, vp, vp, vp, ci, ci, ci, ci, ci, ci, ci, ci, ci, ci, ci, vp]
            L.ds_resize_lanczos.argtypes = [vp, vp, ci, ci, ci, ci, i64, i64, i64, vp, ci, ci, vp, vp, ci, vp, vp, ci, vp, vp]
            L.ds_custom_depth_to_f64.argtypes = [vp, vp, ci, ci, ci, ci, i64, i64, i64, ci, vp, vp, vp]
            L.ds_kernel_timer_enable.argtypes = [vp, ci]
            L.ds_kernel_timer_read.argtypes = [vp, ci, ctypes.POINTER(i64), ctypes.POINTER(cd)]
            L.ds_kernel_timer_read_each.argtypes = [vp, ci, ctypes.POINTER(ctypes.c_float), i64, ctypes.POINTER(i64)]
            L.ds_profile_enable.argtypes = [vp, ci]
            L.ds_profile_last_ms.argtypes = [vp, ctypes.POINTER(ctypes.c_float), ctypes.POINTER(ctypes.c_float)]
            for name in EXPORTS:
                getattr(L, name)
            _lib = L
    return _lib


def _check(rc):
    if rc != 0:
        raise DepthStereoError(f"libdepthstereo_hip error {rc}: {lib().ds_last_error().decode(errors='replace')}")


_ctxs = {}


def ctx_for(device_index):
    key = (threading.get_ident(), int(device_index))
    c = _ctxs.get(key)
    if c is None:
        h = ctypes.c_void_p()
        _check(lib().ds_ctx_create(ctypes.byref(h), int(device_index)))
        _ctxs[key] = c = h
    return c


def _torch():
    import torch
    return torch


def require_gpu():
    torch = _torch()
    if not torch.cuda.is_available():
        raise DepthStereoError("no MI355X visible to torch (torch.cuda.is_available() is False); "
                               "this package has no CPU path")
    return torch


def _stream(t):
    torch = _torch()
    return ctypes.c_void_p(torch.cuda.current_stream(t.device).cuda_stream)


def _dev_index(t):
    torch = _torch()
    return t.device.index if t.device.index is not None else torch.cuda.current_device()


def _depth_dtype_id(t):
    torch = _torch()
    if t.dtype in (torch.uint16, torch.int16):
        return DS_DEPTH_U16
    if t.dtype == torch.float32:
        return DS_DEPTH_F32
    if t.dtype == torch.float64:
        return DS_DEPTH_F64
    raise DepthStereoError(f"unsupported device depth dtype {t.dtype}")


def depth_minmax(depth):
    torch = require_gpu()
    n, h, w = depth.shape
    out = torch.empty((n, 2), dtype=torch.float64, device=depth.device)
    CALLS["ds_depth_minmax"] += 1
    _check(lib().ds_depth_minmax(ctx_for(_dev_index(depth)), depth.data_ptr(), _depth_dtype_id(depth), n, h, w,
                                 out.data_ptr(), _stream(depth)))
    return out


def build_pow_lut(depth_u16, exponent):
    torch = require_gpu()
    mm = depth_minmax(depth_u16).cpu().numpy()
    n = mm.shape[0]
    lut = np.zeros((n, 65536), np.float64)
    codes = np.arange(65536, dtype=np.float64)
    for i in range(n):
        mn, mx = mm[i]
        if not mx > mn:
            lut[i, :] = np.nan
            continue
        norm = (codes - mn) / (mx - mn)
        lo, hi = int(mn), int(mx)
        vals = [math.pow(x, exponent) for x in norm[lo:hi + 1].tolist()]
        lut[i, lo:hi + 1] = vals
    return torch.from_numpy(lut).to(depth_u16.device)


def stereo_warp(image, depth, eyes, fill, exponent=1.0, pow_lut=None):
    require_gpu()
    assert image.is_contiguous() and depth.is_contiguous()
    n, h, w, c = image.shape
    arr = (ds_eye * len(eyes))()
    for i, (dv, sp, ptr, rs, is_) in enumerate(eyes):
        arr[i].divergence_px = float(dv)
        arr[i].separation_px = float(sp)
        arr[i].out = ptr
        arr[i].out_row_stride = int(rs)
        arr[i].out_img_stride = int(is_)
    CALLS["ds_stereo_warp"] += 1
    _check(lib().ds_stereo_warp(ctx_for(_dev_index(image)), image.data_ptr(), depth.data_ptr(), _depth_dtype_id(depth),
                                n, h, w, c, float(exponent), pow_lut.data_ptr() if pow_lut is not None else None,
                                FILL_IDS[fill], arr, len(eyes), _stream(image)))


def last_exact_rows(image):
    v = ctypes.c_int64(0)
    _check(lib().ds_stereo_last_exact_rows(ctx_for(_dev_index(image)), ctypes.byref(v), _stream(image)))
    return int(v.value)


def last_stats(image):
    v = (ctypes.c_int64 * 2)()
    _check(lib().ds_stereo_last_stats(ctx_for(_dev_index(image)), v, _stream(image)))
    return int(v[0]), int(v[1])


def profile_enable(device_index, enable=True):
    _check(lib().ds_profile_enable(ctx_for(device_index), 1 if enable else 0))


def profile_last_ms(device_index):
    a, b = ctypes.c_float(0), ctypes.c_float(0)
    _check(lib().ds_profile_last_ms(ctx_for(device_index), ctypes.byref(a), ctypes.byref(b)))
    return float(a.value), float(b.value)


def copy_view(src_ptr, src_rs, src_is, dst_ptr, dst_rs, dst_is, n, h, row_bytes, like):
    CALLS["ds_copy_view"] += 1
    _check(lib().ds_copy_view(ctx_for(_dev_index(like)), src_ptr, src_rs, src_is, dst_ptr, dst_rs, dst_is, n, h, row_bytes,
                              _stream(like)))


def overlap_red_cyan(im1_ptr, r1, i1, im2_ptr, r2, i2, n, h, w, c, out):
    CALLS["ds_overlap_red_cyan"] += 1
    _check(lib().ds_overlap_red_cyan(ctx_for(_dev_index(out)), im1_ptr, r1, i1, im2_ptr, r2, i2, n, h, w, c, out.data_ptr(),
                                     _stream(out)))


def normalmap(depth, pre_blur, sobel_ksize, post_blur, invert, wrap=False):
    torch = require_gpu()
    n, h, w = depth.shape
    assert depth.dtype in (torch.uint16, torch.float64, torch.float32, torch.float16) and depth.is_contiguous()
    out = torch.empty((n, h, w, 3), dtype=torch.uint8, device=depth.device)
    pre_blur, sobel_ksize, post_blur = int(pre_blur), int(sobel_ksize), int(post_blur)
    if depth.dtype == torch.float16:
        assert pre_blur == 0 and post_blur == 0 and sobel_ksize == 0, "float16 depth: np.gradient without blurs only"
        name, sizes = "ds_normalmap_gradient_f16", ()
    elif depth.dtype == torch.float32:
        assert sobel_ksize == 0, "float32 depth: np.gradient only (cv2.Sobel is fed float64)"
        if pre_blur == 0 and post_blur == 0:
            name, sizes = "ds_normalmap_gradient_f32", ()
        else:
            name, sizes = "ds_normalmap_gradient_blur_f32", (pre_blur, post_blur)
    else:
        name, sizes = ("ds_normalmap" if depth.dtype == torch.uint16 else "ds_normalmap_f64"), (pre_blur, sobel_ksize, post_blur)
    if wrap:
        name += "_wrap"
    CALLS[name] += 1
    _check(getattr(lib(), name)(ctx_for(_dev_index(depth)), depth.data_ptr(), n, h, w, *sizes, 1 if invert else 0,
                                out.data_ptr(), _stream(depth)))
    return out


_BILATERAL_TABLES = collections.OrderedDict()
_BILATERAL_TABLES_MAX = 4
_BILATERAL_LOCK = threading.Lock()


def bilateral_params(bilateral):
    try:
        d, sigma_color, sigma_space = bilateral
        ok = not isinstance(d, bool) and int(d) == d
        d, sigma_color, sigma_space = int(d), float(sigma_color), float(sigma_space)
    except (TypeError, ValueError, OverflowError):
        raise ValueError("bilateral must be (d, sigma_color, sigma_space), got %r" % (bilateral,)) from None
    if not (ok and d % 2 == 1 and 3 <= d <= 31):
        raise ValueError("bilateral: d must be an odd integer in 3..31, got %r" % (bilateral[0],))
    if not (0.0 < sigma_color < math.inf and 0.0 < sigma_space < math.inf):
        raise ValueError("bilateral: sigma_color and sigma_space must be finite and > 0, got %r, %r" % (sigma_color, sigma_space))
    return d, sigma_color, sigma_space


def bilateral_tables(d, sigma_color, sigma_space):
    r = d // 2
    dy, dx = np.mgrid[-r:r + 1, -r:r + 1]
    ws = np.where(dx * dx + dy * dy <= r * r, np.exp(-(dx * dx + dy * dy) / (2.0 * sigma_space**2)), 0.0).astype(np.float64).ravel()
    wr = np.exp(-(np.arange(65536, dtype=np.float64)**2) / (2.0 * sigma_color**2))
    return ws, wr


def bilateral_u16(depth_u16, d, sigma_color, sigma_space, wrap=False):
    torch = require_gpu()
    try:
        d, sigma_color, sigma_space = bilateral_params((d, sigma_color, sigma_space))
    except ValueError as e:
        raise DepthStereoError("bilateral_u16: %s" % e) from None
    if not (torch.is_tensor(depth_u16) and depth_u16.is_cuda and depth_u16.dtype == torch.uint16 and depth_u16.dim() == 3):
        raise DepthStereoError("bilateral_u16: depth must be a uint16 cuda tensor [n,h,w] (the range table is indexed by an integer "
                               "difference), got %s %s" % (getattr(depth_u16, "dtype", type(depth_u16)), tuple(getattr(depth_u16, "shape", ()))))
    depth_u16 = depth_u16.contiguous()
    n, h, w = depth_u16.shape
    if not wrap and d // 2 >= min(h, w):
        raise DepthStereoError("bilateral_u16: d // 2 = %d must be below min(h, w) = %d without wrap" % (d // 2, min(h, w)))
    key = (_dev_index(depth_u16), d, sigma_color, sigma_space)
    with _BILATERAL_LOCK:
        tabs = _BILATERAL_TABLES.get(key)
        if tabs is None:
            ws, wr = bilateral_tables(d, sigma_color, sigma_space)
            tabs = _BILATERAL_TABLES[key] = (torch.from_numpy(ws).to(depth_u16.device), torch.from_numpy(wr).to(depth_u16.device))
            while len(_BILATERAL_TABLES) > _BILATERAL_TABLES_MAX:
                _BILATERAL_TABLES.popitem(last=False)
        else:
            _BILATERAL_TABLES.move_to_end(key)
    for t in tabs:
        t.record_stream(torch.cuda.current_stream(depth_u16.device))
    out = torch.empty((n, h, w), dtype=torch.float64, device=depth_u16.device)
    CALLS["ds_bilateral_u16"] += 1
    _check(lib().ds_bilateral_u16(ctx_for(_dev_index(depth_u16)), depth_u16.data_ptr(), n, h, w, d // 2, tabs[0].data_ptr(),
                                  tabs[1].data_ptr(), 1 if wrap else 0, out.data_ptr(), _stream(depth_u16)))
    return out


def depth_to_u16(pred_f32, invert=False, want_norm=False):
    torch = require_gpu()
    n, h, w = pred_f32.shape
    out = torch.empty((n, h, w), dtype=torch.uint16, device=pred_f32.device)
    norm = torch.empty((n, h, w), dtype=torch.float32, device=pred_f32.device) if want_norm else None
    CALLS["ds_depth_to_u16"] += 1
    _check(lib().ds_depth_to_u16(ctx_for(_dev_index(pred_f32)), pred_f32.data_ptr(), n, h, w, 1 if invert else 0,
                                 out.data_ptr(), norm.data_ptr() if want_norm else None, _stream(pred_f32)))
    return (out, norm) if want_norm else out


def convert_to_i16(arr):
    torch = require_gpu()
    assert arr.dtype in (torch.float32, torch.float64) and arr.is_contiguous()
    out = torch.empty(arr.shape, dtype=torch.uint16, device=arr.device)
    CALLS["ds_convert_to_i16"] += 1
    _check(lib().ds_convert_to_i16(ctx_for(_dev_index(arr)), arr.data_ptr(), 1 if arr.dtype == torch.float64 else 0,
                                   arr.numel(), out.data_ptr(), _stream(arr)))
    return out


CD_WIDEN, CD_SINGLE_BAND, CD_MULTI_BAND = 0, 1, 2
_CD_WORKSPACE_BLOCKS = 256
_coeff_cache = collections.OrderedDict()


def _pixel_plane(src):
    torch = _torch()
    from . import resample_model as rm
    pix = {torch.uint8: rm.PIX_U8, torch.uint16: rm.PIX_U16, torch.int32: rm.PIX_I32, torch.float32: rm.PIX_F32}.get(src.dtype)
    if pix is None or not src.is_cuda or not src.is_contiguous() or src.dim() not in (3, 4) or (src.dim() == 4 and pix != rm.PIX_U8):
        raise DepthStereoError(f"unsupported pixel tensor: dtype {src.dtype}, shape {tuple(src.shape)}")
    n, h, w = src.shape[:3]
    c = src.shape[3] if src.dim() == 4 else 1
    return pix, n, h, w, c, w * c, h * w * c


def _lanczos_coeffs_on(device, fixed_point, in_size, out_size):
    torch = _torch()
    from . import resample_model as rm
    key = (str(device), bool(fixed_point), int(in_size), int(out_size))
    hit = _coeff_cache.get(key)
    if hit is None:
        taps, bounds, kk = rm.lanczos_coeffs(int(in_size), int(out_size))
        if fixed_point:
            kk = rm.fixed_point_coeffs(kk)
        hit = (torch.from_numpy(np.array(bounds)).to(device), torch.from_numpy(np.array(kk.T, order='C')).to(device), taps)
        _coeff_cache[key] = hit
        while len(_coeff_cache) > 32:
            _coeff_cache.popitem(last=False)
    else:
        _coeff_cache.move_to_end(key)
    return hit


def resize_lanczos(src, out_hw):
# ... 300 lines not shown
    _check(lib().ds_add_relu_f32(ctx_for(_dev_index(a)), a.data_ptr(), b.data_ptr(), out.data_ptr(), a.numel(), _stream(a)))
    return out


def bias_act_f32_ok(x, bias, res=None):
    torch = require_gpu()
    if not (x.is_cuda and x.dtype == torch.float32 and bias is not None and bias.dtype == torch.float32 and bias.is_cuda and bias.numel() == x.shape[1]):
        return False
    if not (x.dim() == 4 and x.shape[1] % 4 == 0 and x.is_contiguous(memory_format=torch.channels_last) and x.numel() > 0):
        return False
    return res is None or (res.dtype == torch.float32 and res.shape == x.shape and res.is_cuda and res.is_contiguous(memory_format=torch.channels_last))


def bias_act_f32(x, bias, relu=False, res=None):
    assert bias_act_f32_ok(x, bias, res)
    b, c, h, w = x.shape
    bias = bias.contiguous()
    CALLS["ds_bias_act_f32"] += 1
    _check(lib().ds_bias_act_f32(ctx_for(_dev_index(x)), x.data_ptr(), bias.data_ptr(), None if res is None else res.data_ptr(), x.data_ptr(),
                                 b * h * w, c, 1 if relu else 0, _stream(x)))
    return x


def _relu_cat_layout(a, b):
    torch = require_gpu()
    if not (a.is_cuda and b.is_cuda and a.dtype == torch.float32 and b.dtype == torch.float32 and a.dim() == 4 and b.dim() == 4
            and a.shape[0] == b.shape[0] and a.shape[2:] == b.shape[2:] and a.numel() > 0 and b.numel() > 0):
        return None
    cl = torch.channels_last
    if b.is_contiguous():
        lay = 2 if (a.is_contiguous() and not a.is_contiguous(memory_format=cl)) else (1 if a.is_contiguous(memory_format=cl) else None)
        if lay is not None and a.shape[1] % 32 == 0 and b.shape[1] % 32 == 0:
            return lay
    if a.is_contiguous(memory_format=cl) and b.is_contiguous(memory_format=cl) and a.shape[1] % 4 == 0 and b.shape[1] % 4 == 0:
        return 0
    return None


def relu_cat_f32_ok(a, b):
    return _relu_cat_layout(a, b) is not None


def relu_cat_f32(a, b):
    torch = require_gpu()
    lay = _relu_cat_layout(a, b)
    assert lay is not None
    n, ca, h, w = a.shape
    cb = b.shape[1]
    out = torch.empty((n, ca + cb, h, w), dtype=a.dtype, device=a.device, memory_format=torch.channels_last if lay == 0 else torch.contiguous_format)
    CALLS["ds_relu_cat_f32"] += 1
    _check(lib().ds_relu_cat_f32(ctx_for(_dev_index(a)), a.data_ptr(), b.data_ptr(), out.data_ptr(), n, h * w, ca, cb, lay, _stream(a)))
    return out


def dwconv(x, w_taps, bias_in, bias, kernel, stride, pad_top, pad_left, out_hw):
    torch = require_gpu()
    assert x.is_cuda and x.dtype in (torch.float16, torch.float32) and x.dim() == 4
    x = x.contiguous(memory_format=torch.channels_last)
    b, c, h, w = x.shape
    for t, n in ((w_taps, kernel * kernel * c), (bias_in, c), (bias, c)):
        assert t.is_cuda and t.dtype == torch.float32 and t.is_contiguous() and t.numel() == n
    out = torch.empty((b, c, int(out_hw[0]), int(out_hw[1])), dtype=x.dtype, device=x.device, memory_format=torch.channels_last)
    CALLS["ds_dwconv_nhwc"] += 1
    _check(lib().ds_dwconv_nhwc(ctx_for(_dev_index(x)), x.data_ptr(), w_taps.data_ptr(), bias_in.data_ptr(), bias.data_ptr(), out.data_ptr(),
                                b, h, w, c, out.shape[2], out.shape[3], int(kernel), int(stride), int(pad_top), int(pad_left),
                                1 if x.dtype == torch.float16 else 3, _stream(x)))
    return out


KT_KINDS = {"linear_gelu": 0, "attention": 1, "linear_residual": 2, "linear": 3, "linear_vt": 4, "conv3x3": 5, "linear_readout": 6,
            "linear_shuffle": 7, "normalmap": 8}
KT_RAGGED = 12


def kernel_timer_enable(device_index, enable=True):
    _check(lib().ds_kernel_timer_enable(ctx_for(device_index), 1 if enable else 0))


def kernel_timer_read(device_index, kind):
    base, _, rag = kind.partition("+")
    k = KT_KINDS[base] + (KT_RAGGED if rag == "ragged" else 0)
    n, ms = ctypes.c_int64(), ctypes.c_double()
    _check(lib().ds_kernel_timer_read(ctx_for(device_index), k, ctypes.byref(n), ctypes.byref(ms)))
    return int(n.value), float(ms.value)


def kernel_timer_read_each(device_index, kind):
    base, _, rag = kind.partition("+")
    k = KT_KINDS[base] + (KT_RAGGED if rag == "ragged" else 0)
    buf = (ctypes.c_float * 1024)()
    n = ctypes.c_int64()
    _check(lib().ds_kernel_timer_read_each(ctx_for(device_index), k, buf, 1024, ctypes.byref(n)))
    return [float(buf[i]) for i in range(min(int(n.value), 1024))]


def row_stats(x, eps):
    torch = require_gpu()
    assert x.is_cuda and x.dtype in (torch.float16, torch.bfloat16) and x.is_contiguous()
    c = x.shape[-1]
    rows = x.numel() // c
    out = torch.empty((rows, 2), dtype=torch.float32, device=x.device)
    CALLS["ds_row_stats"] += 1
    _check(lib().ds_row_stats(ctx_for(_dev_index(x)), x.data_ptr(), out.data_ptr(), rows, c, float(eps),
                              1 if x.dtype == torch.float16 else 2, _stream(x)))
    return out


def linear_ln(x, w_scaled, colsum, bias, stats, gelu=False):
    torch = require_gpu()
    assert x.is_cuda and x.dtype in (torch.float16, torch.bfloat16) and linear_supported(x, w_scaled) and x.is_contiguous()
    k, n = x.shape[-1], w_scaled.shape[0]
    rows = x.numel() // k
    assert rows >= 256 and w_scaled.dtype == x.dtype and w_scaled.is_contiguous() and colsum.dtype == torch.float32 and colsum.numel() == n
    assert stats.dtype == torch.float32 and stats.numel() == 2 * rows and (bias is None or (bias.dtype == x.dtype and bias.is_contiguous()))
    out = torch.empty((rows, n), dtype=x.dtype, device=x.device)
    CALLS["ds_linear_ln"] += 1
    _check(lib().ds_linear_ln(ctx_for(_dev_index(x)), x.data_ptr(), w_scaled.data_ptr(), colsum.data_ptr(), None if bias is None else bias.data_ptr(),
                              stats.data_ptr(), out.data_ptr(), rows, n, k, n, 1 if gelu else 0, 1 if x.dtype == torch.float16 else 2, _stream(x)))
    return out.view(x.shape[:-1] + (n,))


def linear_vt_ln(w_v_scaled, colsum, x, stats):
    torch = require_gpu()
    assert x.is_cuda and x.dtype in (torch.float16, torch.bfloat16) and linear_vt_supported(w_v_scaled, x) and x.is_contiguous()
    b, npad, k = x.shape
    c = w_v_scaled.shape[0]
    assert w_v_scaled.dtype == x.dtype and w_v_scaled.is_contiguous() and colsum.dtype == torch.float32 and colsum.numel() == c
    assert stats.dtype == torch.float32 and stats.numel() == 2 * b * npad
    out = torch.empty((b, c, npad), dtype=x.dtype, device=x.device)
    CALLS["ds_linear_vt_ln"] += 1
    _check(lib().ds_linear_vt_ln(ctx_for(_dev_index(x)), w_v_scaled.data_ptr(), colsum.data_ptr(), x.data_ptr(), stats.data_ptr(), out.data_ptr(),
                                 c, b, npad, k, 1 if x.dtype == torch.float16 else 2, _stream(x)))
    return out


def linear_vt_supported(w_v, h):
    return (h.dim() == 3 and h.shape[1] % 8 == 0 and (h.shape[0] * h.shape[1]) % 256 == 0 and w_v.shape[0] >= 256
            and w_v.shape[1] == h.shape[2] and h.shape[2] % 128 == 0 and 128 <= h.shape[2] <= 16384
            and h.shape[0] * h.shape[1] * h.shape[1] < (1 << 32))


def linear_vt(w_v, h):
    torch = require_gpu()
    assert h.is_cuda and h.dtype in (torch.float16, torch.bfloat16) and linear_vt_supported(w_v, h)
    b, npad, k = h.shape
    c = w_v.shape[0]
    h2 = h if h.is_contiguous() else h.contiguous()
    w = w_v.detach()
    w = w if (w.dtype == h.dtype and w.is_contiguous()) else w.to(h.dtype).contiguous()
    out = torch.empty((b, c, npad), dtype=h.dtype, device=h.device)
    CALLS["ds_linear_vt"] += 1
    _check(lib().ds_linear_vt(ctx_for(_dev_index(h)), w.data_ptr(), h2.data_ptr(), out.data_ptr(), c, b, npad, k,
                              1 if h.dtype == torch.float16 else 2, _stream(h)))
    return out


def linear_qkv_supported(h, w_qk, w_v):
    return linear_vt_supported(w_v, h) and linear_supported(h, w_qk) and w_qk.shape[1] == h.shape[2]


def linear_qkv(h, w_qk, b_qk, w_v, out=None):
    torch = require_gpu()
    assert h.is_cuda and h.dtype in (torch.float16, torch.bfloat16) and linear_qkv_supported(h, w_qk, w_v)
    b, npad, k = h.shape
    n, c = w_qk.shape[0], w_v.shape[0]
    h2 = h if h.is_contiguous() else h.contiguous()

    def prep(t):
        if t is None:
            return None
        t = t.detach()
        return t if (t.dtype == h.dtype and t.is_contiguous()) else t.to(h.dtype).contiguous()
    wq, bq, wv = prep(w_qk), prep(b_qk), prep(w_v)
    if out is None:
        qk = torch.empty((b, npad, n), dtype=h.dtype, device=h.device)
        vt = torch.empty((b, c, npad), dtype=h.dtype, device=h.device)
    else:
        qk, vt = out
        assert tuple(qk.shape) == (b, npad, n) and tuple(vt.shape) == (b, c, npad) and qk.is_contiguous() and vt.is_contiguous()
        assert qk.dtype == vt.dtype == h.dtype and qk.device == vt.device == h.device
    CALLS["ds_linear_qkv"] += 1
    CALLS["ds_linear"] += 1
    CALLS["ds_linear_vt"] += 1
    _check(lib().ds_linear_qkv(ctx_for(_dev_index(h)), h2.data_ptr(), wq.data_ptr(), None if bq is None else bq.data_ptr(), wv.data_ptr(),
                               qk.data_ptr(), vt.data_ptr(), b, npad, n, c, k, 1 if h.dtype == torch.float16 else 2, _stream(h)))
    return qk, vt


def conv3x3_supported(conv, x):
    return (tuple(conv.kernel_size) == (3, 3) and tuple(conv.stride) == (1, 1) and tuple(conv.padding) == (1, 1)
            and tuple(conv.dilation) == (1, 1) and conv.groups == 1 and conv.padding_mode == 'zeros'
            and conv.in_channels % 128 == 0 and conv.out_channels % 128 == 0 and x.dim() == 4 and x.shape[1] == conv.in_channels
            and x.shape[0] * x.shape[2] * x.shape[3] >= 256)


def conv3x3_circular_supported(conv, x):
    return (tuple(conv.kernel_size) == (3, 3) and tuple(conv.stride) == (1, 1) and tuple(conv.padding) == (1, 1)
            and tuple(conv.dilation) == (1, 1) and conv.groups == 1 and conv.padding_mode == 'circular'
            and conv.in_channels % 128 == 0 and conv.out_channels % 128 == 0 and x.dim() == 4 and x.shape[1] == conv.in_channels
            and x.shape[0] * x.shape[2] * x.shape[3] >= 256)


def conv3x3(conv, x, relu=False, res1=None, res2=None, relu_in=False):
    torch = require_gpu()
    circular = conv.padding_mode == 'circular'
    assert x.is_cuda and x.dtype in (torch.float16, torch.bfloat16)
    assert conv3x3_circular_supported(conv, x) if circular else conv3x3_supported(conv, x)
    x = x.contiguous(memory_format=torch.channels_last)
    b, c, h, w = x.shape
    key = (conv.weight.data_ptr(), conv.weight._version, x.dtype, None if conv.bias is None else conv.bias._version)
    hit = getattr(conv, "_ds_ohwi", None)
    if hit is None or hit[0] != key:
        if hit is not None:
            from . import vit_mi355x as _vm
            _vm.cache_evicted()
        wk = conv.weight.detach().to(x.dtype).permute(0, 2, 3, 1).contiguous()
        bk = None if conv.bias is None else conv.bias.detach().to(x.dtype).contiguous()
        hit = conv._ds_ohwi = (key, wk, bk)
    _, wk, bk = hit
    out = torch.empty((b, conv.out_channels, h, w), dtype=x.dtype, device=x.device, memory_format=torch.channels_last)
    for r in (res1, res2):
        assert r is None or (r.shape == out.shape and r.dtype == x.dtype and r.is_contiguous(memory_format=torch.channels_last))
    name = "ds_conv3x3_nhwc_circular" if circular else "ds_conv3x3_nhwc"
    CALLS[name] += 1
    _check(getattr(lib(), name)(ctx_for(_dev_index(x)), x.data_ptr(), wk.data_ptr(), None if bk is None else bk.data_ptr(),
                                None if res1 is None else res1.data_ptr(), None if res2 is None else res2.data_ptr(),
                                out.data_ptr(), b, h, w, c, conv.out_channels, (2 if relu else 0) | (4 if relu_in else 0),
                                1 if x.dtype == torch.float16 else 2, _stream(x)))
    return out


def bias_act(x, bias, relu=False, res1=None, res2=None, inplace=True):
    torch = require_gpu()
    assert x.is_cuda and x.dtype in (torch.float16, torch.bfloat16) and x.dim() == 4 and x.shape[1] % 8 == 0
    assert x.is_contiguous(memory_format=torch.channels_last)
    for r in (res1, res2):
        assert r is None or (r.shape == x.shape and r.dtype == x.dtype and r.is_contiguous(memory_format=torch.channels_last))
    out = x if inplace else torch.empty_like(x)
    b = bias.detach().to(x.dtype).contiguous()
    CALLS["ds_bias_act_nhwc"] += 1
    _check(lib().ds_bias_act_nhwc(ctx_for(_dev_index(x)), x.data_ptr(), b.data_ptr(), None if res1 is None else res1.data_ptr(),
                                  None if res2 is None else res2.data_ptr(), out.data_ptr(), x.numel(), x.shape[1], 1 if relu else 0,
                                  1 if x.dtype == torch.float16 else 2, _stream(x)))
    return out


def group_norm_supported(x, groups):
    torch = _torch()
    return (x.is_cuda and x.dtype in (torch.float16, torch.bfloat16) and x.dim() == 4 and x.is_contiguous() and x.shape[1] % groups == 0
            and (x.shape[2] * x.shape[3]) % 8 == 0 and x.shape[0] * groups <= 4096 and x.data_ptr() % 16 == 0)


def group_norm(x, groups, weight, bias, eps, relu=False, res=None):
    torch = require_gpu()
    assert group_norm_supported(x, groups)
    assert res is None or (res.shape == x.shape and res.dtype == x.dtype and res.is_contiguous() and res.data_ptr() % 16 == 0)
    out = torch.empty_like(x)
    g, b = weight.detach().to(x.dtype).contiguous(), bias.detach().to(x.dtype).contiguous()
    CALLS["ds_group_norm_nchw"] += 1
    _check(lib().ds_group_norm_nchw(ctx_for(_dev_index(x)), x.data_ptr(), g.data_ptr(), b.data_ptr(), None if res is None else res.data_ptr(),
                                    out.data_ptr(), x.shape[0], x.shape[1], x.shape[2] * x.shape[3], int(groups), float(eps), 1 if relu else 0,
                                    1 if x.dtype == torch.float16 else 2, _stream(x)))
    return out


def boost_blend(dst, rects, coefs, preds, mask_template):
    torch = require_gpu()
    assert dst.is_cuda and dst.dtype == torch.float32 and dst.dim() == 2 and dst.stride(1) == 1
    n = len(rects)
    if n == 0:
        return dst
    preds = preds.contiguous()
    mask_template = mask_template.contiguous()
    assert preds.dtype == torch.float32 and preds.shape[0] == n and preds.shape[1] == preds.shape[2]
    assert mask_template.dtype == torch.float32 and mask_template.shape[0] == mask_template.shape[1]
    rec = np.zeros(n, dtype=[('x0', '<i4'), ('y0', '<i4'), ('w', '<i4'), ('h', '<i4'), ('p0', '<f8'), ('p1', '<f8')])
    for i, (r, c) in enumerate(zip(rects, coefs)):
        rec[i] = (int(r[0]), int(r[1]), int(r[2]), int(r[3]), float(c[0]), float(c[1]))
    buf = torch.from_numpy(rec.view(np.uint8).copy()).to(dst.device)
    CALLS["ds_boost_blend"] += 1
    _check(lib().ds_boost_blend(ctx_for(_dev_index(dst)), dst.data_ptr(), dst.stride(0), dst.shape[0], dst.shape[1],
                                buf.data_ptr(), n, preds.data_ptr(), preds.shape[1], mask_template.data_ptr(),
                                mask_template.shape[0], _stream(dst)))
    return dst


def preprocess_bicubic(images_u8, size_hw, mean, std, flip=True, dtype=None):
    torch = require_gpu()
    assert images_u8.is_cuda and images_u8.dtype == torch.uint8 and images_u8.dim() == 4 and images_u8.shape[3] == 3
    dtype = torch.float32 if dtype is None else dtype
    code = {torch.float16: 1, torch.bfloat16: 2, torch.float32: 3}[dtype]
    x = images_u8.contiguous()
    b, h, w, _ = x.shape
    oh, ow = int(size_hw[0]), int(size_hw[1])
    out = torch.empty((b, 3, oh, ow), dtype=dtype, device=x.device, memory_format=torch.channels_last)
    m = (ctypes.c_float * 3)(*[float(v) for v in (mean if hasattr(mean, "__len__") else (mean,) * 3)])
    s = (ctypes.c_float * 3)(*[float(v) for v in (std if hasattr(std, "__len__") else (std,) * 3)])
    CALLS["ds_preprocess_bicubic"] += 1
    _check(lib().ds_preprocess_bicubic(ctx_for(_dev_index(x)), x.data_ptr(), out.data_ptr(), b, h, w, oh, ow, 1 if flip else 0, m, s, code,
                                       _stream(x)))
    return out


def upsample_bilinear(x, size=None, scale_factor=None, align_corners=True):
    torch = require_gpu()
    b, c, ih, iw = x.shape
    if size is None:
        size = (int(ih * scale_factor), int(iw * scale_factor))
    oh, ow = int(size[0]), int(size[1])
    assert x.is_cuda and x.dtype in (torch.float16, torch.bfloat16) and c % 8 == 0
    xin = x.contiguous(memory_format=torch.channels_last)
    out = torch.empty((b, c, oh, ow), dtype=x.dtype, device=x.device, memory_format=torch.channels_last)
    CALLS["ds_upsample_bilinear_nhwc"] += 1
    _check(lib().ds_upsample_bilinear_nhwc(ctx_for(_dev_index(x)), xin.data_ptr(), out.data_ptr(), b, c, ih, iw, oh, ow,
                                           1 if align_corners else 0, 1 if x.dtype == torch.float16 else 2, _stream(x)))
    return out


def dpt_head_tail(x, size, conv3, conv1, relu_out=True):
    torch = require_gpu()
    b, c, ih, iw = x.shape
    assert c == 128 and tuple(conv3.weight.shape) == (32, 128, 3, 3) and tuple(conv1.weight.shape) == (1, 32, 1, 1)
    xin = x.contiguous(memory_format=torch.channels_last)
    key = tuple((p.data_ptr(), p._version) for p in (conv3.weight, conv3.bias, conv1.weight, conv1.bias)) + (x.dtype, x.device)
    hit = getattr(conv3, "_ds_head_cache", None)
    if hit is None or hit[0] != key:
        if hit is not None:
            from . import vit_mi355x as _vm
            _vm.cache_evicted()
        w = conv3.weight.detach().to(x.dtype)
        wf = w.permute(2, 3, 1, 0).reshape(9, 8, 2, 8, 32).permute(0, 1, 2, 4, 3).contiguous()
        hit = (key, wf, conv3.bias.detach().float().contiguous(), conv1.weight.detach().float().reshape(32).contiguous(),
               float(conv1.bias.detach().float().item()))
        conv3._ds_head_cache = hit
    _, wf, b2, w3, b3 = hit
    oh, ow = int(size[0]), int(size[1])
    out = torch.empty((b, 1, oh, ow), dtype=x.dtype, device=x.device)
    assert conv3.padding_mode in ('zeros', 'circular') and tuple(conv3.padding) == (1, 1)
    name = "ds_dpt_head_tail_circular" if conv3.padding_mode == 'circular' else "ds_dpt_head_tail"
    CALLS[name] += 1
    _check(getattr(lib(), name)(ctx_for(_dev_index(x)), xin.data_ptr(), b, ih, iw, oh, ow, wf.data_ptr(), b2.data_ptr(),
                                w3.data_ptr(), b3, 1 if relu_out else 0, out.data_ptr(),
                                1 if x.dtype == torch.float16 else 2, _stream(x)))
    return out
```

stable-diffusion-webui-depthmap-script_amd/src/vit_mi355x.py:

```python
import contextlib
import functools
import math
import os
import threading

import torch
import torch.nn as nn
import torch.nn.functional as F

HEAD_DIM = 64
SEQ_ALIGN = 64

_CONSTANTS = {}

CACHE_EPOCH = [0]
SIZE_CACHE_ENTRIES = 6


def cache_evicted():
    CACHE_EPOCH[0] += 1


def cache_store(cache, key, value, entries=None):
    if len(cache) >= (SIZE_CACHE_ENTRIES if entries is None else entries):
# ... 52 lines not shown
        q1 = min(npad, q0 + rows)
        att = (q[:, :, q0:q1] * scale) @ kt
        if bias is not None:
            bt = bias.rows(q0, q1) if hasattr(bias, "rows") else bias[:, q0:q1]
            att = att + bt.to(ct).unsqueeze(0)
        if n_valid < npad:
            att[..., n_valid:] = float('-inf')
        outs.append(att.softmax(dim=-1) @ v)
    out = outs[0] if len(outs) == 1 else torch.cat(outs, dim=2)
    return out.permute(0, 2, 1, 3).reshape(b, npad, h * d).to(qk.dtype)


def v_transposed(w_v, h):
    b = h.shape[0]
    if half_on_gpu(h) and LINEAR_HIP == "all":
        from . import _native
        if _native.linear_vt_supported(w_v, h) and hip_gemm_ok(w_v.shape[0], h.shape[0] * h.shape[1]):
            return _native.linear_vt(w_v, h)
    return torch.bmm(w_v.unsqueeze(0).expand(b, -1, -1), h.transpose(1, 2))


def folded_proj_bias(proj, b_v):
    if b_v is None:
        return proj.bias
    key = (proj.weight._version, proj.bias._version, b_v._version, b_v.data_ptr(), proj.weight.data_ptr(), proj.weight.dtype)
    hit = getattr(proj, "_folded_bias", None)
    if hit is not None and hit[0] == key:
        return hit[1]
    out = proj.bias + F.linear(b_v.to(proj.weight.dtype), proj.weight)
    if not torch.is_grad_enabled():
        if hit is not None:
            cache_evicted()
        proj._folded_bias = (key, out)
    return out


LOG2E = 1.4426950408889634


LINEAR_HIP = os.environ.get("DS_LINEAR", "all")


LINEAR_HIP_MIN_TILES = int(os.environ.get("DS_LINEAR_MIN_TILES", 96))


def hip_gemm_ok(rows, out_features):
    return rows >= 256 and ((rows + 255) // 256) * (out_features // 256) >= LINEAR_HIP_MIN_TILES


LINEAR_QKV = os.environ.get("DS_LINEAR_QKV", "1") != "0"


def linear_qkv_ok(h, w_qk, w_v):
    if not (LINEAR_QKV and LINEAR_HIP == "all" and half_on_gpu(h) and h.dim() == 3):
        return False
    from . import _native
    rows = h.shape[0] * h.shape[1]
    return (_native.linear_qkv_supported(h, w_qk, w_v) and hip_gemm_ok(rows, w_qk.shape[0]) and hip_gemm_ok(w_v.shape[0], rows))


STOCK = [False]


def half_on_gpu(x):
    return x.is_cuda and x.dtype in (torch.float16, torch.bfloat16) and not STOCK[0]


@contextlib.contextmanager
def stock_routing():
    saved = STOCK[0]
    STOCK[0] = True
    try:
        yield
    finally:
        STOCK[0] = saved


DETERMINISTIC_LIBRARY = os.environ.get("DS_DETERMINISTIC", "0") == "1"
INVARIANT = os.environ.get("DS_INVARIANT", "1") != "0"
_size_routed = threading.local()


def invariant():
    return INVARIANT and not getattr(_size_routed, "depth", 0)


@contextlib.contextmanager
def size_routed():
    _size_routed.depth = getattr(_size_routed, "depth", 0) + 1
    try:
        yield
    finally:
        _size_routed.depth -= 1
_det_lock = threading.Lock()
_det_state = [0, False]


@contextlib.contextmanager
def deterministic_library():
    if not DETERMINISTIC_LIBRARY:
        yield
        return
    with _det_lock:
        if _det_state[0] == 0:
            _det_state[1] = torch.backends.cudnn.deterministic
            torch.backends.cudnn.deterministic = True
        _det_state[0] += 1
    try:
        yield
    finally:
        with _det_lock:
            _det_state[0] -= 1
            if _det_state[0] == 0:
                torch.backends.cudnn.deterministic = _det_state[1]


def deterministic_forward(fn):
    @functools.wraps(fn)
    def wrapped(*args, **kwargs):
        with deterministic_library():
            return fn(*args, **kwargs)
    return wrapped


@contextlib.contextmanager
def library_routing():
    global LINEAR_HIP, CONV_HIP
    saved = LINEAR_HIP, CONV_HIP
    LINEAR_HIP, CONV_HIP = "0", False
    try:
        yield
    finally:
        LINEAR_HIP, CONV_HIP = saved


def linear(x, weight, bias=None, gelu=False):
    if half_on_gpu(x) and (LINEAR_HIP == "all" or (gelu and LINEAR_HIP in ("gelu", "proj"))):
        from . import _native
        if _native.linear_supported(x, weight) and (gelu or hip_gemm_ok(x.numel() // x.shape[-1], weight.shape[0])):
            return _native.linear(x, weight, bias, gelu)
    y = F.linear(x, weight, bias)
    return F.gelu(y) if gelu else y


def fused_attention(qk, vt, n_valid, scale, bias=None):
    if qk.dtype in (torch.float32, torch.float64) or STOCK[0]:
        return attention_reference(qk, vt, n_valid, scale, bias)
    from . import _native
    return _native.attention_fwd(qk, vt, n_valid, scale, bias)


class EncoderBlock(nn.Module):

    def __init__(self, dim, num_heads, mlp_ratio=4.0):
        super().__init__()
        assert dim == num_heads * HEAD_DIM, "the attention kernel is built for head_dim 64"
        self.dim, self.num_heads = dim, num_heads
        self.scale = HEAD_DIM ** -0.5

    def attention_bias(self, n_pad, grid_hw, dtype, device):
        return None

    def attend_o(self, h, n_valid, grid_hw):
        b, npad, c = h.shape
        w_qk, b_qk, w_v, b_v = self.qkv_weights()
        if linear_qkv_ok(h, w_qk, w_v):
            from . import _native
            qk, vt = _native.linear_qkv(h, w_qk, b_qk, w_v)
            qk = qk.view(b, npad, 2, self.num_heads, HEAD_DIM)
        else:
            qk = linear(h, w_qk, b_qk).view(b, npad, 2, self.num_heads, HEAD_DIM)
            vt = v_transposed(w_v, h)
        return fused_attention(qk, vt, n_valid, self.scale, self.attention_bias(npad, grid_hw, h.dtype, h.device)), b_v

    def attend(self, h, n_valid, grid_hw):
        o, b_v = self.attend_o(h, n_valid, grid_hw)
        return self.proj(o, b_v)

    def forward_padded(self, x, n_valid, grid_hw=None):
        g1, g2 = self.gammas()
        a = self.attend(self.norm1(x), n_valid, grid_hw)
        x = x + (a if g1 is None else g1 * a)
        m = self.mlp(self.norm2(x))
        return x + (m if g2 is None else g2 * m)


LN_FOLD = os.environ.get("DS_LN_FOLD", "0") != "0"
LN_FOLD_CHANNELS = (384, 768, 1024, 1536)


def _ln_fold_params(blk, dtype):
    w_qk, b_qk, w_v, b_v = blk.qkv_weights()
    n1, n2, fc1, pr = blk.norm1, blk.norm2, blk.mlp.fc1, blk.attn.proj
    tensors = (w_qk, b_qk, w_v, b_v, n1.weight, n1.bias, n2.weight, n2.bias, fc1.weight, fc1.bias, pr.weight, pr.bias)
    key = tuple((None if t is None else (t._version, t.data_ptr())) for t in tensors) + (dtype,)
    hit = getattr(blk, "_ln_fold", None)
    if hit is not None and hit[0] == key:
        return hit[1]
    if hit is not None:
        cache_evicted()

    def fold(w, b, ln):
        wf = w.float()
        ws = (wf * ln.weight.float()[None, :]).to(dtype).contiguous()
        const = wf @ ln.bias.float() + (0.0 if b is None else b.float())
        return ws, ws.float().sum(1).contiguous(), const
    wqk, sqk, cqk = fold(w_qk, b_qk, n1)
    wv, sv, cv = fold(w_v, b_v, n1)
    w1, s1, c1 = fold(fc1.weight, fc1.bias, n2)
    pb = ((0.0 if pr.bias is None else pr.bias.float()) + pr.weight.float() @ cv).to(dtype).contiguous()
    out = {"wqk": wqk, "sqk": sqk, "bqk": cqk.to(dtype).contiguous(), "wv": wv, "sv": sv, "proj_bias": pb,
           "w1": w1, "s1": s1, "b1": c1.to(dtype).contiguous()}
    if not torch.is_grad_enabled():
        blk._ln_fold = (key, out)
    return out


def _ln_fold_ok(blocks, x):
    if not (LN_FOLD and LINEAR_HIP == "all" and half_on_gpu(x) and x.is_contiguous() and x.shape[2] in LN_FOLD_CHANNELS):
        return False
    from . import _native
    rows = x.shape[0] * x.shape[1]
    if not hip_gemm_ok(rows, x.shape[2]):
        return False
    for blk in blocks:
        mlp, pr = getattr(blk, "mlp", None), getattr(getattr(blk, "attn", None), "proj", None)
        if not (isinstance(mlp, Mlp) and pr is not None and mlp.fc2.bias is not None and hasattr(blk, "qkv_weights")
                and isinstance(getattr(blk, "norm1", None), nn.LayerNorm) and isinstance(getattr(blk, "norm2", None), nn.LayerNorm)
                and blk.norm1.elementwise_affine and blk.norm2.elementwise_affine and blk.norm1.bias is not None and blk.norm2.bias is not None):
            return False
        w_qk, _, w_v, _ = blk.qkv_weights()
        if not (_native.linear_supported(x, w_qk) and _native.linear_supported(x, pr.weight) and _native.linear_supported(x, mlp.fc1.weight)
                and mlp.fc2.weight.shape[0] % 256 == 0 and mlp.fc2.weight.shape[1] % 128 == 0 and _native.linear_vt_supported(w_v, x)):
            return False
    return True


def _run_blocks_ln_fold(blocks, x, n_valid, grid_hw, take, padded_taps):
    from . import _native
    taps = {}
    b, npad, c = x.shape
    for i, blk in enumerate(blocks):
        p = _ln_fold_params(blk, x.dtype)
        g1, g2 = blk.gammas()
        st = _native.row_stats(x, blk.norm1.eps)
        qk = _native.linear_ln(x, p["wqk"], p["sqk"], p["bqk"], st).view(b, npad, 2, blk.num_heads, HEAD_DIM)
        vt = _native.linear_vt_ln(p["wv"], p["sv"], x, st)
        o = fused_attention(qk, vt, n_valid, blk.scale, blk.attention_bias(npad, grid_hw, x.dtype, x.device))
        x = _native.linear_residual(o, blk.attn.proj.weight, p["proj_bias"], g1, x)
        st = _native.row_stats(x, blk.norm2.eps)
        a = _native.linear_ln(x, p["w1"], p["s1"], p["b1"], st, gelu=True)
        x = _native.linear_residual(a, blk.mlp.fc2.weight, blk.mlp.fc2.bias, g2, x)
        if i in take:
            taps[i] = x if padded_taps else x[:, :n_valid]
    return x, taps


def run_blocks(blocks, x, n_valid, grid_hw, take, padded_taps=False):
    taps = {}
    fast = half_on_gpu(x)
    if not fast:
        for i, blk in enumerate(blocks):
            x = blk.forward_padded(x, n_valid, grid_hw)
            if i in take:
                taps[i] = x if padded_taps else x[:, :n_valid]
        return x, taps
    if _ln_fold_ok(blocks, x):
        return _run_blocks_ln_fold(blocks, x, n_valid, grid_hw, take, padded_taps)
    from . import _native
    n = len(blocks)
    _, h = _native.residual_layernorm(x, None, None, blocks[0].norm1.weight, blocks[0].norm1.bias, blocks[0].norm1.eps)
    big = hip_gemm_ok(x.shape[0] * x.shape[1], x.shape[2])
    for i, blk in enumerate(blocks):
        g1, g2 = blk.gammas()
        pr = getattr(getattr(blk, "attn", None), "proj", None)
        if (LINEAR_HIP in ("proj", "all") and pr is not None and big and _native.linear_supported(x, pr.weight)):
            o, b_v = blk.attend_o(h, n_valid, grid_hw)
            x = _native.linear_residual(o, pr.weight, folded_proj_bias(pr, b_v), g1, x)
            _, h2 = _native.residual_layernorm(x, None, None, blk.norm2.weight, blk.norm2.bias, blk.norm2.eps)
        else:
            p = blk.attend(h, n_valid, grid_hw)
            x, h2 = _native.residual_layernorm(x, p, g1, blk.norm2.weight, blk.norm2.bias, blk.norm2.eps)
        mlp = blk.mlp
        fused_fc2 = (LINEAR_HIP == "all" and isinstance(mlp, Mlp) and big and _native.linear_supported(x, mlp.fc2.weight)
                     and _native.linear_supported(h2, mlp.fc1.weight) and mlp.fc2.bias is not None)
        if fused_fc2:
            a = _native.linear(h2, mlp.fc1.weight, mlp.fc1.bias, True)
            x = _native.linear_residual(a, mlp.fc2.weight, mlp.fc2.bias, g2, x)
            if i + 1 < n:
                nxt = blocks[i + 1].norm1
                _, h = _native.residual_layernorm(x, None, None, nxt.weight, nxt.bias, nxt.eps)
        else:
            m = mlp(h2)
            if i + 1 < n:
                nxt = blocks[i + 1].norm1
                x, h = _native.residual_layernorm(x, m, g2, nxt.weight, nxt.bias, nxt.eps)
            else:
                x = x + (m if g2 is None else g2 * m)
        if i in take:
            taps[i] = x if padded_taps else x[:, :n_valid]
    return x, taps


def interpolate_bilinear(x, size=None, scale_factor=None, align_corners=True):
    if half_on_gpu(x) and x.shape[1] % 8 == 0:
        from . import _native
        return _native.upsample_bilinear(x, size=size, scale_factor=scale_factor, align_corners=align_corners)
    if size is not None:
        return F.interpolate(x, size=size, mode="bilinear", align_corners=align_corners)
    return F.interpolate(x, scale_factor=scale_factor, mode="bilinear", align_corners=align_corners)


CONV_HIP = os.environ.get("DS_CONV", "1") != "0"
CONV_HIP_MIN_TILES = int(os.environ.get("DS_CONV_MIN_TILES", 48))
CONV_HEAD_HIP = os.environ.get("DS_CONV_HEAD", "1") != "0"
CONV_RELU_IN = os.environ.get("DS_CONV_RELU_IN", "1") != "0"
CONV_CIRCULAR_HIP = os.environ.get("DS_CONV_CIRCULAR", "1") != "0"


def circular_hip_ok(conv):
    return CONV_CIRCULAR_HIP or getattr(conv, "padding_mode", "zeros") != "circular"


def conv3x3_hip_ok(conv, x):
    if not (CONV_HIP and half_on_gpu(x) and x.dim() == 4):
        return False
    from . import _native
    if conv.out_channels % 256 != 0 and not CONV_HEAD_HIP:
        return False
    tiles = (x.shape[0] * x.shape[2] * x.shape[3] + 255) // 256 * ((conv.out_channels + 255) // 256)
    supported = _native.conv3x3_supported(conv, x) or (CONV_CIRCULAR_HIP and _native.conv3x3_circular_supported(conv, x))
    return supported and tiles >= (1 if invariant() else CONV_HIP_MIN_TILES)


def conv2d(conv, x):
    if conv3x3_hip_ok(conv, x):
        from . import _native
        return _native.conv3x3(conv, x)
    return conv(x)


CONV_BIAS_HIP = os.environ.get("DS_CONV_BIAS", "1") != "0"
CONV1X1_HIP = os.environ.get("DS_CONV1X1", "1") != "0"
CONVT_HIP = os.environ.get("DS_CONVT", "1") != "0"
READOUT_HIP = os.environ.get("DS_READOUT", "1") != "0"
CONV1X1_MIN_TILES = int(os.environ.get("DS_CONV1X1_MIN_TILES", 96))


def conv1x1_hip_ok(layer, x):
    if not (CONV1X1_HIP and LINEAR_HIP == "all" and half_on_gpu(x) and x.dim() == 4 and type(layer) is nn.Conv2d):
        return False
    if not (tuple(layer.kernel_size) == (1, 1) and tuple(layer.stride) == (1, 1) and tuple(layer.padding) == (0, 0) and layer.groups == 1
            and tuple(layer.dilation) == (1, 1)):
        return False
    pixels = x.shape[0] * x.shape[2] * x.shape[3]
    return (layer.out_channels % 256 == 0 and layer.in_channels % 128 == 0 and 128 <= layer.in_channels <= 16384 and pixels >= 256
            and ((pixels + 255) // 256) * (layer.out_channels // 256) >= (1 if invariant() else CONV1X1_MIN_TILES)
            and x.is_contiguous(memory_format=torch.channels_last))


def conv1x1(layer, x):
    from . import _native
    b, c, h, w = x.shape
    rows = x.permute(0, 2, 3, 1).reshape(b * h * w, c)
    y = _native.linear(rows, layer.weight.reshape(layer.out_channels, c), layer.bias)
    return y.view(b, h, w, layer.out_channels).permute(0, 3, 1, 2)


def conv_transpose_hip_ok(layer, x):
    if not (CONVT_HIP and LINEAR_HIP == "all" and half_on_gpu(x) and x.dim() == 4 and type(layer) is nn.ConvTranspose2d):
        return False
    from . import _native
    if not (_native.conv_transpose_shuffle_supported(layer, x) and x.is_contiguous(memory_format=torch.channels_last)):
        return False
    pixels = x.shape[0] * x.shape[2] * x.shape[3]
    n = layer.stride[0] * layer.stride[0] * layer.out_channels
    return ((pixels + 255) // 256) * (n // 256) >= (1 if invariant() else CONV1X1_MIN_TILES)


def _gemm_weight(layer, x, kpad):
    w = layer.weight
    key = (w.data_ptr(), w._version, x.dtype, kpad)
    cache = getattr(layer, "_ds_gemm_weight", None)
    if cache is None or cache[0] != key:
        wm = w.detach().permute(0, 2, 3, 1).reshape(w.shape[0], -1).to(x.dtype)
        if wm.shape[1] != kpad:
            wm = torch.cat([wm, wm.new_zeros((wm.shape[0], kpad - wm.shape[1]))], 1)
        cache = (key, wm.contiguous())
        layer._ds_gemm_weight = cache
    return cache[1]


def patch_embed_hip_ok(conv, x):
    if not (invariant() and LINEAR_HIP == "all" and half_on_gpu(x) and x.dim() == 4 and type(conv) is nn.Conv2d):
        return False
    k = conv.kernel_size
    return (k[0] == k[1] and tuple(conv.stride) == tuple(k) and tuple(conv.padding) == (0, 0) and conv.groups == 1
            and tuple(conv.dilation) == (1, 1) and conv.out_channels % 256 == 0 and x.shape[1] == conv.in_channels
            and x.shape[2] >= k[0] and x.shape[3] >= k[1] and x.is_contiguous(memory_format=torch.channels_last))


def patch_embed_tokens(conv, x):
    from . import _native
    b, c, h, w = x.shape
    p = conv.kernel_size[0]
    gh, gw = h // p, w // p
    k = p * p * c
    kpad = (k + 127) // 128 * 128
    xv = x.permute(0, 2, 3, 1)[:, :gh * p, :gw * p].reshape(b, gh, p, gw, p, c).permute(0, 1, 3, 2, 4, 5)
    if kpad == k:
        rows = xv.reshape(b * gh * gw, k)
    else:
        rows = x.new_zeros((b * gh * gw, kpad))
        rows[:, :k] = xv.reshape(b * gh * gw, k)
    y = _native.linear(rows, _gemm_weight(conv, x, kpad), conv.bias)
    return y.view(b, gh * gw, conv.out_channels)


def strided3x3_hip_ok(layer, x):
    if not (invariant() and LINEAR_HIP == "all" and half_on_gpu(x) and x.dim() == 4 and type(layer) is nn.Conv2d):
        return False
    return (tuple(layer.kernel_size) == (3, 3) and tuple(layer.stride) == (2, 2) and tuple(layer.padding) == (1, 1) and layer.groups == 1
            and tuple(layer.dilation) == (1, 1) and layer.out_channels % 256 == 0
            and (layer.padding_mode == "zeros" or (layer.padding_mode == "circular" and CONV_CIRCULAR_HIP))
            and layer.in_channels % 128 == 0 and 9 * layer.in_channels <= 16384 and x.shape[1] == layer.in_channels)


def conv_strided3x3(layer, x):
    from . import _native
    b, c, h, w = x.shape
    ho, wo = (h - 1) // 2 + 1, (w - 1) // 2 + 1
    xp = F.pad(x, (1, 1, 1, 1), mode="circular") if layer.padding_mode == "circular" else F.pad(x, (1, 1, 1, 1))
    xp = xp.permute(0, 2, 3, 1).contiguous()
    sb, sh, sw, sc = xp.stride()
    rows = xp.as_strided((b, ho, wo, 3, 3, c), (sb, 2 * sh, 2 * sw, sh, sw, sc)).reshape(b * ho * wo, 9 * c)
    y = _native.linear(rows, _gemm_weight(layer, x, 9 * c), layer.bias)
    return y.view(b, ho, wo, layer.out_channels).permute(0, 3, 1, 2)
PREPROCESS_HIP = os.environ.get("DS_PREPROCESS", "1") != "0"


def conv_module(layer, x):
    if conv1x1_hip_ok(layer, x):
        return conv1x1(layer, x)
    if strided3x3_hip_ok(layer, x):
        return conv_strided3x3(layer, x)
    if conv_transpose_hip_ok(layer, x):
        from . import _native
        return _native.conv_transpose_shuffle(layer, x)
    if (CONV_BIAS_HIP and half_on_gpu(x) and x.dim() == 4 and getattr(layer, "bias", None) is not None
            and layer.out_channels % 8 == 0 and getattr(layer, "padding_mode", "zeros") == "zeros"):
        if type(layer) is nn.Conv2d:
            y = layer._conv_forward(x, layer.weight, None)
        elif type(layer) is nn.ConvTranspose2d:
            y = F.conv_transpose2d(x, layer.weight, None, layer.stride, layer.padding, layer.output_padding, layer.groups, layer.dilation)
        else:
            return layer(x)
        if y.is_contiguous(memory_format=torch.channels_last):
            from . import _native
            return _native.bias_act(y, layer.bias, relu=False)
        return y + layer.bias.view(1, -1, 1, 1)
    return layer(x)


def residual_conv_unit(conv1, conv2, x, skip=None):
    if (half_on_gpu(x) and x.shape[1] % 8 == 0 and conv1.bias is not None
            and conv2.bias is not None and conv1.out_channels % 8 == 0):
        from . import _native
        xc = x.contiguous(memory_format=torch.channels_last)
        if (conv3x3_hip_ok(conv1, xc) and conv3x3_hip_ok(conv2, xc) and conv1.out_channels == conv2.in_channels
                and conv2.out_channels % 256 == 0):
            sk = None if skip is None else skip.contiguous(memory_format=torch.channels_last)
            if CONV_RELU_IN and conv1.out_channels % 256 == 0:
                a = _native.conv3x3(conv1, xc, relu=True, relu_in=True)
            else:
                a = _native.conv3x3(conv1, F.relu(xc), relu=True)
            return _native.conv3x3(conv2, a, relu=False, res1=xc, res2=sk)
        c1 = conv1._conv_forward(F.relu(xc), conv1.weight, None)
        if c1.is_contiguous(memory_format=torch.channels_last):
            a = _native.bias_act(c1, conv1.bias, relu=True)
            c2 = conv2._conv_forward(a, conv2.weight, None)
            if c2.is_contiguous(memory_format=torch.channels_last) and c2.shape == xc.shape:
                sk = None if skip is None else skip.contiguous(memory_format=torch.channels_last)
                return _native.bias_act(c2, conv2.bias, relu=False, res1=xc, res2=sk)
            out = c2 + conv2.bias.view(1, -1, 1, 1) + x
            return out if skip is None else skip + out
        out = conv2(F.relu(c1 + conv1.bias.view(1, -1, 1, 1))) + x
        return out if skip is None else skip + out
    out = conv1(F.relu(x))
    out = conv2(F.relu(out))
    out = out + x
    return out if skip is None else skip + out


class Mlp(nn.Module):

    def __init__(self, dim, hidden):
        super().__init__()
        self.fc1 = nn.Linear(dim, hidden)
        self.fc2 = nn.Linear(hidden, dim)

    def forward(self, x):
        return linear(linear(x, self.fc1.weight, self.fc1.bias, gelu=True), self.fc2.weight, self.fc2.bias)


def count_encoder_flops(depth, n, dim, mlp_ratio=4.0):
    lin = 2.0 * (4.0 + 2.0 * mlp_ratio) * n * dim * dim
    att = 4.0 * n * n * dim
    return depth * (lin + att)
```

Measured before the change: 898.8 pairs/s.

## Fuse preprocessing into patch rows, add bicubic tail and im2col kernels

Adds a kernel that resizes the u8 image bicubically, normalises it and writes patch-embedding GEMM rows directly, replacing separate resize, normalise and patch-gather steps. A token fixup kernel then writes the cls token and zeroes the padding rows. Two more kernels are added: a bicubic upsample of the depth prediction that writes f32 directly, and a native im2col for the strided 3x3 convolutions that replaces pad, permute and as_strided copies. The goal is fewer launches and less intermediate memory traffic at the two ends of the forward pass, at the cost of more custom code that must match the reference numerics.

```diff
diff --git a/include/depthstereo.h b/include/depthstereo.h
--- a/include/depthstereo.h
+++ b/include/depthstereo.h
@@ -214,6 +214,18 @@
                    int n_patches, const float *preds, int pred_size, const float *mask_template, int mask_size,
                    void *stream);
 
+int ds_preprocess_bicubic_rows(ds_ctx *ctx, const void *images, void *rows, int batch, int in_h, int in_w, int out_h, int out_w,
+                               int flip_channels, const float *mean, const float *std, int patch, int n_pad, int kpad, int dtype,
+                               void *stream);
+
+int ds_tokens_fixup(ds_ctx *ctx, void *tokens, const void *cls, int batch, int n_pad, int n_valid, int channels, int dtype, void *stream);
+
+int ds_upsample_bicubic_to_f32(ds_ctx *ctx, const void *in, void *out, int batch, int in_h, int in_w, int out_h, int out_w, int dtype,
+                               void *stream);
+
+int ds_im2col3x3_s2_nhwc(ds_ctx *ctx, const void *x, void *rows, int batch, int height, int width, int channels, int circular, int dtype,
+                         void *stream);
+
 #ifdef __cplusplus
 }
 #endif
diff --git a/stable-diffusion-webui-depthmap-script_amd/build_native.py b/stable-diffusion-webui-depthmap-script_amd/build_native.py
--- a/stable-diffusion-webui-depthmap-script_amd/build_native.py
+++ b/stable-diffusion-webui-depthmap-script_amd/build_native.py
@@ -8,7 +8,7 @@
 EXPERIMENTS = bool(os.environ.get("DS_EXPERIMENTS"))
 OUT = os.path.join(HERE, "libdepthstereo_hip_experiments.so" if EXPERIMENTS else "libdepthstereo_hip.so")
 OBJ_DIR = os.path.join(HERE, "build", "experiments") if EXPERIMENTS else os.path.join(HERE, "build")
-SOURCES = ["ds_api.hip", "ds_stereo.hip", "ds_stereo_polylines.hip", "ds_normalmap.hip", "ds_attention.hip", "ds_attention4.hip", "ds_encoder_ops.hip", "ds_boost.hip", "ds_heatmap.hip", "ds_linear.hip", "ds_gconv.hip", "ds_dwconv.hip", "ds_resample.hip", "ds_bilateral.hip"]
+SOURCES = ["ds_api.hip", "ds_stereo.hip", "ds_stereo_polylines.hip", "ds_normalmap.hip", "ds_attention.hip", "ds_attention4.hip", "ds_encoder_ops.hip", "ds_forward_ends.hip", "ds_boost.hip", "ds_heatmap.hip", "ds_linear.hip", "ds_gconv.hip", "ds_dwconv.hip", "ds_resample.hip", "ds_bilateral.hip"]
 FLAGS = ["--offload-arch=gfx950", "-O3", "-std=c++17", "-ffp-contract=off", "-fno-fast-math", "-fPIC",
          "-fvisibility=hidden", "-Wall", "-Wno-unused-function",
          "-mllvm", "-amdgpu-mfma-vgpr-form=1"]
diff --git a/stable-diffusion-webui-depthmap-script_amd/csrc/ds_common.h b/stable-diffusion-webui-depthmap-script_amd/csrc/ds_common.h
--- a/stable-diffusion-webui-depthmap-script_amd/csrc/ds_common.h
+++ b/stable-diffusion-webui-depthmap-script_amd/csrc/ds_common.h
@@ -79,6 +79,16 @@
 __device__ __forceinline__ int ds_wrap_prev(int i, int n) { return i > 0 ? i - 1 : n - 1; }
 __device__ __forceinline__ int ds_wrap_next(int i, int n) { return i + 1 < n ? i + 1 : 0; }
 
+__device__ __forceinline__ void pre_cubic(float t, float *c)
+{
+    const float A = -0.75f;
+    const float x0 = t + 1.0f, x3 = 2.0f - t, x2 = 1.0f - t;
+    c[0] = ((A * x0 - 5.0f * A) * x0 + 8.0f * A) * x0 - 4.0f * A;
+    c[1] = ((A + 2.0f) * t - (A + 3.0f)) * t * t + 1.0f;
+    c[2] = ((A + 2.0f) * x2 - (A + 3.0f)) * x2 * x2 + 1.0f;
+    c[3] = ((A * x3 - 5.0f * A) * x3 + 8.0f * A) * x3 - 4.0f * A;
+}
+
 __device__ __forceinline__ double ds_wave_min(double v)
 {
     for (int o = 32; o > 0; o >>= 1) { double t = __shfl_xor(v, o, 64); v = t < v ? t : v; }
diff --git a/stable-diffusion-webui-depthmap-script_amd/csrc/ds_encoder_ops.hip b/stable-diffusion-webui-depthmap-script_amd/csrc/ds_encoder_ops.hip
--- a/stable-diffusion-webui-depthmap-script_amd/csrc/ds_encoder_ops.hip
+++ b/stable-diffusion-webui-depthmap-script_amd/csrc/ds_encoder_ops.hip
@@ -239,16 +239,6 @@
     float mean[3], istd[3];
     long long total;
 };
-
-__device__ __forceinline__ void pre_cubic(float t, float *c)
-{
-    const float A = -0.75f;
-    const float x0 = t + 1.0f, x3 = 2.0f - t, x2 = 1.0f - t;
-    c[0] = ((A * x0 - 5.0f * A) * x0 + 8.0f * A) * x0 - 4.0f * A;
-    c[1] = ((A + 2.0f) * t - (A + 3.0f)) * t * t + 1.0f;
-    c[2] = ((A + 2.0f) * x2 - (A + 3.0f)) * x2 * x2 + 1.0f;
-    c[3] = ((A * x3 - 5.0f * A) * x3 + 8.0f * A) * x3 - 4.0f * A;
-}
 
 template <int DT>
 __global__ __launch_bounds__(256) void k_preprocess_bicubic(PreParams P)
diff --git a/stable-diffusion-webui-depthmap-script_amd/csrc/ds_forward_ends.hip b/stable-diffusion-webui-depthmap-script_amd/csrc/ds_forward_ends.hip
--- /dev/null
+++ b/stable-diffusion-webui-depthmap-script_amd/csrc/ds_forward_ends.hip
@@ -0,0 +1,397 @@
+#include <algorithm>
+
+#include "ds_common.h"
+
+template <int BF16> struct fe_traits;
+template <> struct fe_traits<0> { typedef _Float16 T; };
+template <> struct fe_traits<1> { typedef __bf16 T; };
+
+#define FE_ROWS_MAX 160
+#define FE_P_MAX 32
+struct RowsParams {
+    const uint8_t *in, *in_end;
+    const uint8_t *safe;
+    void *rows;
+    int ih, iw, flip;
+    float sy, sx, mean[3], istd[3];
+    int p, gh, gw, n_pad, kpad, twp;
+    int src_rows, src_pitch;
+    int region;
+};
+
+__device__ __forceinline__ float fe_u8_unit(uint8_t v)
+{
+    const float r = 1.0f / 255.0f, x = (float)v, q = x * r;
+    return __builtin_fmaf(__builtin_fmaf(-q, 255.0f, x), r, q);
+}
+
+template <int BF16>
+__global__ __launch_bounds__(256) void k_preprocess_rows(RowsParams P)
+{
+    typedef typename fe_traits<BF16>::T T;
+    extern __shared__ uint4 fe_smem[];
+    const int tid = threadIdx.x, lane = tid & 63, wv = tid >> 6;
+    const int b = blockIdx.z, gy = blockIdx.y, C8 = P.kpad >> 3;
+    uint4 *rows = (uint4 *)P.rows + (size_t)b * P.n_pad * C8;
+    const uint4 z4 = make_uint4(0, 0, 0, 0);
+    if (gy == P.gh) {
+        const int nz = P.n_pad - P.gh * P.gw;
+        for (int z = blockIdx.x; z < nz; z += gridDim.x) {
+            uint4 *dst = rows + (size_t)(z == 0 ? 0 : P.gh * P.gw + z) * C8;
+            for (int i = tid; i < C8; i += 256) dst[i] = z4;
+        }
+        return;
+    }
+    const int gx0 = blockIdx.x * P.twp, np = min(P.twp, P.gw - gx0), npx = np * P.p, K = 3 * P.p * P.p;
+    unsigned char *sm = (unsigned char *)fe_smem;
+    int *xs = (int *)sm;                       sm += 64 * 4 * sizeof(int);
+    float *cxs = (float *)sm;                  sm += 64 * 4 * sizeof(float);
+    int *ys = (int *)sm;                       sm += FE_P_MAX * 4 * sizeof(int);
+    float *cys = (float *)sm;                  sm += FE_P_MAX * 4 * sizeof(float);
+    int *colmeta = (int *)sm;                  sm += 64 * sizeof(int);
+    unsigned char *src = sm;
+    T *otile = (T *)sm;                        sm += P.region;
+    float *hbuf = (float *)sm;
+
+    if (tid < npx) {
+        const float fx = P.sx * ((float)(gx0 * P.p + tid) + 0.5f) - 0.5f, fx0 = floorf(fx);
+        float c[4];
+        pre_cubic(fx - fx0, c);
+        const int ix = (int)fx0;
+#pragma unroll
+        for (int k = 0; k < 4; k++) { xs[tid * 4 + k] = min(max(ix - 1 + k, 0), P.iw - 1); cxs[tid * 4 + k] = c[k]; }
+        const int pj = tid / P.p;
+        colmeta[tid] = pj * P.kpad + (tid - pj * P.p) * 3;
+    } else if (tid >= 64 && tid < 64 + P.p) {
+        const int py = tid - 64;
+        const float fy = P.sy * ((float)(gy * P.p + py) + 0.5f) - 0.5f, fy0 = floorf(fy);
+        float c[4];
+        pre_cubic(fy - fy0, c);
+        const int iy = (int)fy0;
+#pragma unroll
+        for (int k = 0; k < 4; k++) { ys[py * 4 + k] = min(max(iy - 1 + k, 0), P.ih - 1); cys[py * 4 + k] = c[k]; }
+    }
+    __syncthreads();
+    const int x_lo = xs[0], x_hi = xs[(npx - 1) * 4 + 3], y_lo = ys[0], y_hi = ys[(P.p - 1) * 4 + 3];
+    const int nrows = y_hi - y_lo + 1, nbytes = (x_hi - x_lo + 1) * 3;
+    const uint8_t *img = P.in + (size_t)b * P.ih * P.iw * 3;
+    const bool staged = nrows <= P.src_rows && nbytes + 30 <= P.src_pitch;
+    int xo[4];
+    float cx[4];
+    if (lane < npx) {
+#pragma unroll
+        for (int k = 0; k < 4; k++) { xo[k] = xs[lane * 4 + k]; cx[k] = cxs[lane * 4 + k]; }
+    }
+    if (staged) {
+        const int nch = P.src_pitch >> 4, total = nrows * nch;
+        for (int base = tid; base < total; base += 1024) {
+            uint4 v[4];
+            const uint8_t *s[4];
+            bool whole[4], part[4];
+#pragma unroll
+            for (int u = 0; u < 4; u++) {
+                const int i = min(base + u * 256, total - 1);
+                const int r = (int)((unsigned)i / (unsigned)nch), c = i - r * nch;
+                const uint8_t *a = img + ((size_t)(y_lo + r) * P.iw + x_lo) * 3;
+                const int sh = (int)((uintptr_t)a & 15);
+                s[u] = a - sh + 16 * c;
+                const bool need = 16 * c < sh + nbytes;
+                whole[u] = need && s[u] >= P.in && s[u] + 16 <= P.in_end;
+                part[u] = need && !whole[u];
+                v[u] = *(const uint4 *)(whole[u] ? s[u] : P.safe);
+            }
+#pragma unroll
+            for (int u = 0; u < 4; u++) {
+                if (part[u]) {
+                    unsigned char t[16];
+#pragma unroll
+                    for (int k = 0; k < 16; k++) t[k] = (s[u] + k >= P.in && s[u] + k < P.in_end) ? s[u][k] : (unsigned char)0;
+                    __builtin_memcpy(&v[u], t, 16);
+                }
+                if (base + u * 256 < total) ((uint4 *)src)[base + u * 256] = v[u];
+            }
+        }
+        __syncthreads();
+        if (lane < npx) {
+            for (int r = wv; r < nrows; r += 4) {
+                const int sh = (int)((uintptr_t)(img + ((size_t)(y_lo + r) * P.iw + x_lo) * 3) & 15);
+                const unsigned char *row = src + (size_t)r * P.src_pitch + sh;
+                float h[3] = {0.f, 0.f, 0.f};
+#pragma unroll
+                for (int kx = 0; kx < 4; kx++) {
+                    const unsigned char *px = row + (xo[kx] - x_lo) * 3;
+#pragma unroll
+                    for (int c = 0; c < 3; c++) h[c] += cx[kx] * fe_u8_unit(px[c]);
+                }
+                float *hh = hbuf + (r * 64 + lane) * 3;
+                hh[0] = h[0]; hh[1] = h[1]; hh[2] = h[2];
+            }
+        }
+        __syncthreads();
+    }
+    for (int i = tid; i < np * (P.kpad - K); i += 256) {
+        const int pj = i / (P.kpad - K);
+        otile[pj * P.kpad + K + (i - pj * (P.kpad - K))] = (T)0.f;
+    }
+    if (lane < npx) {
+        const int cm = colmeta[lane];
+        for (int py = wv; py < P.p; py += 4) {
+            float acc[3] = {0.f, 0.f, 0.f};
+#pragma unroll
+            for (int ky = 0; ky < 4; ky++) {
+                const int y = ys[py * 4 + ky];
+                const float cy = cys[py * 4 + ky];
+                float h[3];
+                if (staged) {
+                    const float *hh = hbuf + ((y - y_lo) * 64 + lane) * 3;
+                    h[0] = hh[0]; h[1] = hh[1]; h[2] = hh[2];
+                } else {
+                    const uint8_t *row = img + (size_t)y * P.iw * 3;
+                    h[0] = h[1] = h[2] = 0.f;
+#pragma unroll
+                    for (int kx = 0; kx < 4; kx++) {
+                        const uint8_t *px = row + (size_t)xo[kx] * 3;
+#pragma unroll
+                        for (int c = 0; c < 3; c++) h[c] += cx[kx] * fe_u8_unit(px[c]);
+                    }
+                }
+#pragma unroll
+                for (int c = 0; c < 3; c++) acc[c] += cy * h[c];
+            }
+            T *q = otile + cm + py * P.p * 3;
+#pragma unroll
+            for (int c = 0; c < 3; c++) q[c] = (T)((acc[P.flip ? 2 - c : c] - P.mean[c]) * P.istd[c]);
+        }
+    }
+    __syncthreads();
+    uint4 *dst = rows + (size_t)(1 + gy * P.gw + gx0) * C8;
+    for (int i = tid; i < np * C8; i += 256) dst[i] = ((const uint4 *)otile)[i];
+}
+
+DS_API int ds_preprocess_bicubic_rows(ds_ctx *ctx, const void *images, void *rows, int batch, int in_h, int in_w, int out_h, int out_w,
+                                      int flip_channels, const float *mean, const float *std, int patch, int n_pad, int kpad,
+                                      int dtype, void *stream)
+{
+    DS_REQUIRE(ctx && images && rows && mean && std, DS_EINVAL, "ds_preprocess_bicubic_rows: null argument");
+    DS_REQUIRE(batch > 0 && in_h > 0 && in_w > 0 && out_h > 0 && out_w > 0, DS_EINVAL, "ds_preprocess_bicubic_rows: bad shape");
+    DS_REQUIRE(dtype == DS_DTYPE_F16 || dtype == DS_DTYPE_BF16, DS_EINVAL, "ds_preprocess_bicubic_rows: dtype must be f16 or bf16");
+    DS_REQUIRE(std[0] != 0.f && std[1] != 0.f && std[2] != 0.f, DS_EINVAL, "ds_preprocess_bicubic_rows: std must be non-zero");
+    DS_REQUIRE(patch >= 1 && patch <= FE_P_MAX && out_h >= patch && out_w >= patch, DS_EINVAL, "ds_preprocess_bicubic_rows: patch size 1..32, at most the output size");
+    const int gh = out_h / patch, gw = out_w / patch;
+    DS_REQUIRE(kpad >= 3 * patch * patch && (kpad % 8) == 0 && (long long)n_pad >= 1 + (long long)gh * gw, DS_EINVAL,
+               "ds_preprocess_bicubic_rows: kpad must be a multiple of 8 that holds 3 * patch^2 values, n_pad at least 1 + the patch count");
+    DS_REQUIRE(((uintptr_t)rows & 15) == 0, DS_EINVAL, "ds_preprocess_bicubic_rows: rows must be 16-byte aligned");
+    DS_REQUIRE(gh + 1 <= 65535 && batch <= 65535 && (long long)batch * in_h * in_w * 3 < (1ll << 46) && (long long)in_h * in_w < (1ll << 29),
+               DS_EUNSUPPORTED, "ds_preprocess_bicubic_rows: tensor too large");
+    DS_HIP_CHECK(hipSetDevice(ctx->device));
+    RowsParams P;
+    P.in = (const uint8_t *)images; P.in_end = P.in + (size_t)batch * in_h * in_w * 3; P.rows = rows;
+    P.ih = in_h; P.iw = in_w; P.flip = flip_channels ? 1 : 0;
+    P.sy = (float)in_h / (float)out_h; P.sx = (float)in_w / (float)out_w;
+    for (int c = 0; c < 3; c++) { P.mean[c] = mean[c]; P.istd[c] = 1.0f / std[c]; }
+    P.p = patch; P.gh = gh; P.gw = gw; P.n_pad = n_pad; P.kpad = kpad;
+    P.twp = 64 / patch;
+    const size_t tables = 64 * 4 * 8 + FE_P_MAX * 4 * 8 + 64 * 4, otile = (size_t)P.twp * kpad * 2;
+    DS_REQUIRE(tables + otile <= 48 * 1024, DS_EUNSUPPORTED, "ds_preprocess_bicubic_rows: kpad too large");
+    const double need_rows = (double)patch * P.sy + 5.0, need_cols = (double)(P.twp * patch) * P.sx + 5.0;
+    size_t lds = tables + otile;
+    P.src_rows = 0; P.src_pitch = 0; P.region = (int)otile;
+    P.safe = (const uint8_t *)(((uintptr_t)P.in + 15) & ~(uintptr_t)15);
+    if (need_rows <= FE_ROWS_MAX && need_cols <= 4096 && P.safe + 16 <= P.in_end) {
+        const int nr = (int)need_rows + 1, pitch = (((int)need_cols + 1) * 3 + 30 + 15) & ~15;
+        const size_t region = std::max(otile, (size_t)nr * pitch);
+        const size_t want = tables + region + (size_t)nr * 64 * 3 * sizeof(float);
+        if (want <= 64 * 1024) { P.src_rows = nr; P.src_pitch = pitch; P.region = (int)region; lds = want; }
+    }
+    dim3 grid((unsigned)((gw + P.twp - 1) / P.twp), (unsigned)(gh + 1), (unsigned)batch);
+    hipStream_t st = (hipStream_t)stream;
+    if (dtype == DS_DTYPE_F16) hipLaunchKernelGGL((k_preprocess_rows<0>), grid, dim3(256), lds, st, P);
+    else hipLaunchKernelGGL((k_preprocess_rows<1>), grid, dim3(256), lds, st, P);
+    DS_HIP_CHECK(hipGetLastError());
+    return DS_OK;
+}
+
+template <int BF16>
+__global__ __launch_bounds__(256) void k_tokens_fixup(void *tokens_, const void *cls_, int n_pad, int n_valid, int C8)
+{
+    const int per = 1 + n_pad - n_valid, b = blockIdx.x / per, k = blockIdx.x - b * per;
+    uint4 *dst = (uint4 *)tokens_ + ((size_t)b * n_pad + (k == 0 ? 0 : n_valid + k - 1)) * C8;
+    const uint4 *cls = (const uint4 *)cls_;
+    for (int i = threadIdx.x; i < C8; i += 256) dst[i] = k == 0 ? cls[i] : make_uint4(0, 0, 0, 0);
+}
+
+DS_API int ds_tokens_fixup(ds_ctx *ctx, void *tokens, const void *cls, int batch, int n_pad, int n_valid, int channels, int dtype,
+                           void *stream)
+{
+    DS_REQUIRE(ctx && tokens && cls, DS_EINVAL, "ds_tokens_fixup: null argument");
+    DS_REQUIRE(batch > 0 && n_valid >= 1 && n_pad >= n_valid && channels > 0 && (channels % 8) == 0, DS_EINVAL,
+               "ds_tokens_fixup: bad shape (channels must be a multiple of 8)");
+    DS_REQUIRE(dtype == DS_DTYPE_F16 || dtype == DS_DTYPE_BF16, DS_EINVAL, "ds_tokens_fixup: dtype must be f16 or bf16");
+    DS_REQUIRE(((uintptr_t)tokens & 15) == 0 && ((uintptr_t)cls & 15) == 0, DS_EINVAL, "ds_tokens_fixup: 16-byte alignment");
+    DS_REQUIRE((long long)batch * (1 + n_pad - n_valid) < (1ll << 31), DS_EUNSUPPORTED, "ds_tokens_fixup: tensor too large");
+    DS_HIP_CHECK(hipSetDevice(ctx->device));
+    dim3 grid((unsigned)(batch * (1 + n_pad - n_valid)));
+    if (dtype == DS_DTYPE_F16) hipLaunchKernelGGL((k_tokens_fixup<0>), grid, dim3(256), 0, (hipStream_t)stream, tokens, cls, n_pad, n_valid, channels / 8);
+    else hipLaunchKernelGGL((k_tokens_fixup<1>), grid, dim3(256), 0, (hipStream_t)stream, tokens, cls, n_pad, n_valid, channels / 8);
+    DS_HIP_CHECK(hipGetLastError());
+    return DS_OK;
+}
+
+#define BT_TH 32
+#define BT_TW 64
+#define BT_SRC_ROWS 40
+#define BT_SRC_COLS 72
+struct TailParams {
+    const void *in;
+    float *out;
+    int ih, iw, oh, ow;
+    float sy, sx;
+};
+
+__device__ __forceinline__ void bt_coeffs(float t, float *c)
+{
+    const float A = -0.75f;
+    const float x1 = t, x0 = x1 + 1.0f, x2 = 1.0f - t, x3 = x2 + 1.0f;
+    c[0] = __builtin_fmaf(__builtin_fmaf(__builtin_fmaf(A, x0, -5.0f * A), x0, 8.0f * A), x0, -4.0f * A);
+    c[1] = __builtin_fmaf(__builtin_fmaf(A + 2.0f, x1, -(A + 3.0f)) * x1, x1, 1.0f);
+    c[2] = __builtin_fmaf(__builtin_fmaf(A + 2.0f, x2, -(A + 3.0f)) * x2, x2, 1.0f);
+    c[3] = __builtin_fmaf(__builtin_fmaf(__builtin_fmaf(A, x3, -5.0f * A), x3, 8.0f * A), x3, -4.0f * A);
+}
+
+template <int FORM>
+__device__ __forceinline__ float bt_interp(float v0, float v1, float v2, float v3, const float *c)
+{
+    if (FORM == 1) return __builtin_fmaf(v3, c[3], __builtin_fmaf(v2, c[2], __builtin_fmaf(v0, c[0], v1 * c[1])));
+    if (FORM == 2) return __builtin_fmaf(v3, c[3], __builtin_fmaf(v2, c[2], __builtin_fmaf(v1, c[1], v0 * c[0])));
+    return v0 * c[0] + v1 * c[1] + v2 * c[2] + v3 * c[3];
+}
+
+template <int BF16>
+__global__ __launch_bounds__(256) void k_upsample_bicubic_f32(TailParams P)
+{
+    typedef typename fe_traits<BF16>::T T;
+    constexpr int NF = BF16 ? 2 : 1;
+    __shared__ int xs[BT_TW * 4], ys[BT_TH * 4];
+    __shared__ float cxs[BT_TW * 4], cys[BT_TH * 4];
+    __shared__ T src[BT_SRC_ROWS * BT_SRC_COLS];
+    __shared__ float hbuf[BT_SRC_ROWS * BT_TW * NF];
+    const int tid = threadIdx.x, lane = tid & 63, wv = tid >> 6, b = blockIdx.z;
+    const int ox0 = blockIdx.x * BT_TW, oy0 = blockIdx.y * BT_TH;
+    const T *in = (const T *)P.in + (size_t)b * P.ih * P.iw;
+    float *out = P.out + (size_t)b * P.oh * P.ow;
+    const int ox = ox0 + lane;
+    if (P.ih == P.oh && P.iw == P.ow) {
+        if (ox < P.ow)
+            for (int oy = oy0 + wv; oy < min(oy0 + BT_TH, P.oh); oy += 4) out[(size_t)oy * P.ow + ox] = (float)in[(size_t)oy * P.iw + ox];
+        return;
+    }
+    if (tid < BT_TW) {
+        const float f = __builtin_fmaf(P.sx, (float)min(ox0 + tid, P.ow - 1) + 0.5f, -0.5f);
+        const int i0 = (int)floorf(f);
+        float c[4];
+        bt_coeffs(f - (float)i0, c);
+#pragma unroll
+        for (int k = 0; k < 4; k++) { xs[tid * 4 + k] = max(min(i0 - 1 + k, P.iw - 1), 0); cxs[tid * 4 + k] = c[k]; }
+    } else if (tid < BT_TW + BT_TH) {
+        const int j = tid - BT_TW;
+        const float f = __builtin_fmaf(P.sy, (float)min(oy0 + j, P.oh - 1) + 0.5f, -0.5f);
+        const int i0 = (int)floorf(f);
+        float c[4];
+        bt_coeffs(f - (float)i0, c);
+#pragma unroll
+        for (int k = 0; k < 4; k++) { ys[j * 4 + k] = max(min(i0 - 1 + k, P.ih - 1), 0); cys[j * 4 + k] = c[k]; }
+    }
+    __syncthreads();
+    const int x_lo = xs[0], x_hi = xs[BT_TW * 4 - 1], y_lo = ys[0], y_hi = ys[BT_TH * 4 - 1];
+    const int nrows = y_hi - y_lo + 1, ncols = x_hi - x_lo + 1;
+    const bool staged = nrows <= BT_SRC_ROWS && ncols <= BT_SRC_COLS;
+    int xo[4];
+    float cx[4];
+#pragma unroll
+    for (int k = 0; k < 4; k++) { xo[k] = xs[lane * 4 + k]; cx[k] = cxs[lane * 4 + k]; }
+    if (staged) {
+        for (int r = wv; r < nrows; r += 4)
+            for (int c = lane; c < ncols; c += 64) src[r * BT_SRC_COLS + c] = in[(size_t)(y_lo + r) * P.iw + x_lo + c];
+        __syncthreads();
+        for (int r = wv; r < nrows; r += 4) {
+            const T *row = src + r * BT_SRC_COLS;
+            const float v0 = (float)row[xo[0] - x_lo], v1 = (float)row[xo[1] - x_lo], v2 = (float)row[xo[2] - x_lo], v3 = (float)row[xo[3] - x_lo];
+            hbuf[(r * BT_TW + lane) * NF] = bt_interp<1>(v0, v1, v2, v3, cx);
+            if (BF16) hbuf[(r * BT_TW + lane) * NF + NF - 1] = bt_interp<2>(v0, v1, v2, v3, cx);
+        }
+        __syncthreads();
+    }
+    if (ox >= P.ow) return;
+    for (int j = wv; j < BT_TH; j += 4) {
+        const int oy = oy0 + j;
+        if (oy >= P.oh) break;
+        float h[4];
+#pragma unroll
+        for (int k = 0; k < 4; k++) {
+            const int y = ys[j * 4 + k];
+            const bool form_b = BF16 && (k & 1);
+            if (staged) {
+                h[k] = hbuf[((y - y_lo) * BT_TW + lane) * NF + (form_b ? 1 : 0)];
+            } else {
+                const T *row = in + (size_t)y * P.iw;
+                const float v0 = (float)row[xo[0]], v1 = (float)row[xo[1]], v2 = (float)row[xo[2]], v3 = (float)row[xo[3]];
+                h[k] = form_b ? bt_interp<2>(v0, v1, v2, v3, cx) : bt_interp<1>(v0, v1, v2, v3, cx);
+            }
+        }
+        const float v = BF16 ? bt_interp<0>(h[0], h[1], h[2], h[3], cys + j * 4) : bt_interp<2>(h[0], h[1], h[2], h[3], cys + j * 4);
+        out[(size_t)oy * P.ow + ox] = (float)(T)v;
+    }
+}
+
+DS_API int ds_upsample_bicubic_to_f32(ds_ctx *ctx, const void *in, void *out, int batch, int in_h, int in_w, int out_h, int out_w,
+                                      int dtype, void *stream)
+{
+    DS_REQUIRE(ctx && in && out, DS_EINVAL, "ds_upsample_bicubic_to_f32: null argument");
+    DS_REQUIRE(batch > 0 && in_h > 0 && in_w > 0 && out_h > 0 && out_w > 0, DS_EINVAL, "ds_upsample_bicubic_to_f32: bad shape");
+    DS_REQUIRE(dtype == DS_DTYPE_F16 || dtype == DS_DTYPE_BF16, DS_EINVAL, "ds_upsample_bicubic_to_f32: dtype must be f16 or bf16");
+    DS_REQUIRE((out_h + BT_TH - 1) / BT_TH <= 65535 && batch <= 65535, DS_EUNSUPPORTED, "ds_upsample_bicubic_to_f32: tensor too large");
+    DS_HIP_CHECK(hipSetDevice(ctx->device));
+    TailParams P;
+    P.in = in; P.out = (float *)out; P.ih = in_h; P.iw = in_w; P.oh = out_h; P.ow = out_w;
+    P.sy = (float)in_h / (float)out_h; P.sx = (float)in_w / (float)out_w;
+    dim3 grid((unsigned)((out_w + BT_TW - 1) / BT_TW), (unsigned)((out_h + BT_TH - 1) / BT_TH), (unsigned)batch);
+    if (dtype == DS_DTYPE_F16) hipLaunchKernelGGL((k_upsample_bicubic_f32<0>), grid, dim3(256), 0, (hipStream_t)stream, P);
+    else hipLaunchKernelGGL((k_upsample_bicubic_f32<1>), grid, dim3(256), 0, (hipStream_t)stream, P);
+    DS_HIP_CHECK(hipGetLastError());
+    return DS_OK;
+}
+
+__global__ __launch_bounds__(256) void k_im2col3x3_s2(const uint4 *in, uint4 *rows, int h, int w, int C8, int circular)
+{
+    const int ox = blockIdx.x, oy = blockIdx.y, b = blockIdx.z, ho = gridDim.y, wo = gridDim.x;
+    uint4 *dst = rows + (((size_t)b * ho + oy) * wo + ox) * 9 * C8;
+    const uint4 *img = in + (size_t)b * h * w * C8;
+    for (int i = threadIdx.x; i < 9 * C8; i += 256) {
+        const int tap = (int)((unsigned)i / (unsigned)C8), c8 = i - tap * C8, ky = tap / 3, kx = tap - ky * 3;
+        int y = 2 * oy + ky - 1, x = 2 * ox + kx - 1;
+        uint4 v = make_uint4(0, 0, 0, 0);
+        if (circular) {
+            y = y < 0 ? h - 1 : (y >= h ? 0 : y);
+            x = x < 0 ? w - 1 : (x >= w ? 0 : x);
+        }
+        if (y >= 0 && y < h && x >= 0 && x < w) v = img[((size_t)y * w + x) * C8 + c8];
+        dst[i] = v;
+    }
+}
+
+DS_API int ds_im2col3x3_s2_nhwc(ds_ctx *ctx, const void *x, void *rows, int batch, int height, int width, int channels, int circular,
+                                int dtype, void *stream)
+{
+    DS_REQUIRE(ctx && x && rows, DS_EINVAL, "ds_im2col3x3_s2_nhwc: null argument");
+    DS_REQUIRE(batch > 0 && height > 0 && width > 0 && channels > 0 && (channels % 8) == 0, DS_EINVAL,
+               "ds_im2col3x3_s2_nhwc: bad shape (channels must be a multiple of 8)");
+    DS_REQUIRE(dtype == DS_DTYPE_F16 || dtype == DS_DTYPE_BF16, DS_EINVAL, "ds_im2col3x3_s2_nhwc: dtype must be f16 or bf16");
+    DS_REQUIRE(((uintptr_t)x & 15) == 0 && ((uintptr_t)rows & 15) == 0, DS_EINVAL, "ds_im2col3x3_s2_nhwc: 16-byte alignment");
+    const int ho = (height - 1) / 2 + 1, wo = (width - 1) / 2 + 1;
+    DS_REQUIRE(ho <= 65535 && batch <= 65535 && 9ll * (channels / 8) < (1ll << 30), DS_EUNSUPPORTED, "ds_im2col3x3_s2_nhwc: tensor too large");
+    DS_HIP_CHECK(hipSetDevice(ctx->device));
+    hipLaunchKernelGGL(k_im2col3x3_s2, dim3((unsigned)wo, (unsigned)ho, (unsigned)batch), dim3(256), 0, (hipStream_t)stream,
+                       (const uint4 *)x, (uint4 *)rows, height, width, channels / 8, circular ? 1 : 0);
+    DS_HIP_CHECK(hipGetLastError());
+    return DS_OK;
+}
diff --git a/stable-diffusion-webui-depthmap-script_amd/dmidas/backbones/beit.py b/stable-diffusion-webui-depthmap-script_amd/dmidas/backbones/beit.py
--- a/stable-diffusion-webui-depthmap-script_amd/dmidas/backbones/beit.py
+++ b/stable-diffusion-webui-depthmap-script_amd/dmidas/backbones/beit.py
@@ -179,6 +179,12 @@
         _, taps = vm.run_blocks(self.blocks, t, n_valid, grid, set(hooks), padded_taps=padded)
         return [taps[i] for i in hooks], grid, n_valid
 
+    def forward_taps_rows(self, rows, grid, hooks, padded=False):
+        n_valid = grid[0] * grid[1] + 1
+        t = vm.patch_rows_tokens(self.patch_embed.proj, self.cls_token, rows, n_valid)
+        _, taps = vm.run_blocks(self.blocks, t, n_valid, grid, set(hooks), padded_taps=padded)
+        return [taps[i] for i in hooks], grid, n_valid
+
 
 class ProjectReadout(nn.Module):
 
@@ -247,8 +253,11 @@
         self.act_postprocess3 = _postprocess(vit_features, f[2], [])
         self.act_postprocess4 = _postprocess(vit_features, f[3], [nn.Conv2d(f[3], f[3], 3, 2, 1)])
 
-    def forward(self, x):
-        taps, grid, n_valid = self.model.forward_taps(x, self.hooks, padded=True)
+    def forward(self, x, rows=None):
+        if rows is not None:
+            taps, grid, n_valid = self.model.forward_taps_rows(rows[0], rows[1], self.hooks, padded=True)
+        else:
+            taps, grid, n_valid = self.model.forward_taps(x, self.hooks, padded=True)
         outs = []
         for tap, post in zip(taps, (self.act_postprocess1, self.act_postprocess2, self.act_postprocess3, self.act_postprocess4)):
             y = post[0].forward_padded(tap, n_valid)
diff --git a/stable-diffusion-webui-depthmap-script_amd/dmidas/dpt_depth.py b/stable-diffusion-webui-depthmap-script_amd/dmidas/dpt_depth.py
--- a/stable-diffusion-webui-depthmap-script_amd/dmidas/dpt_depth.py
+++ b/stable-diffusion-webui-depthmap-script_amd/dmidas/dpt_depth.py
@@ -70,14 +70,14 @@
         scratch.output_conv = head
         self.scratch = scratch
 
-    def forward(self, x, features=None):
+    def forward(self, x, features=None, rows=None):
         if getattr(self, "size_routed", False):
             with vm.size_routed():
-                return self._forward(x, features)
-        return self._forward(x, features)
-
-    def _forward(self, x, features=None):
-        l1, l2, l3, l4 = self.pretrained(x)
+                return self._forward(x, features, rows)
+        return self._forward(x, features, rows)
+
+    def _forward(self, x, features=None, rows=None):
+        l1, l2, l3, l4 = self.pretrained(x) if rows is None else self.pretrained(x, rows=rows)
         s = self.scratch
         l1, l2, l3, l4 = vm.conv2d(s.layer1_rn, l1), vm.conv2d(s.layer2_rn, l2), vm.conv2d(s.layer3_rn, l3), vm.conv2d(s.layer4_rn, l4)
         path_4 = s.refinenet4(l4, size=l3.shape[2:])
@@ -132,6 +132,22 @@
     return _constrain(scale_w * width, multiple), _constrain(scale_h * height, multiple)
 
 
+def _patch_rows(model, images_u8, net_size, net_h, resize_mode, mean, std, dtype):
+    from .backbones.beit import BeitBackbone
+    pre = getattr(model, "pretrained", None)
+    if not (images_u8.is_cuda and isinstance(pre, BeitBackbone)):
+        return None
+    b, h, w, _ = images_u8.shape
+    nw, nh = midas_net_size(w, h, int(net_size), int(net_size if net_h is None else net_h), resize_mode)
+    conv = pre.model.patch_embed.proj
+    if not (vm.patch_rows_ok(conv, dtype, (nh, nw)) and pre.model.cls_token.dtype == dtype):
+        return None
+    from src import _native
+    grid, _, n_pad, kpad = vm.patch_rows_geometry(conv, (nh, nw), b)
+    rows = _native.preprocess_bicubic_rows(images_u8, (nh, nw), mean, std, conv.kernel_size[0], n_pad, kpad, flip=True, dtype=dtype)
+    return rows, grid
+
+
 class DPTDepthModel(DPT):
     def __init__(self, path=None, non_negative=True, **kwargs):
         features = kwargs.get("features", 256)
@@ -156,8 +172,8 @@
         self.load_state_dict(parameters, strict=False)
 
     @vm.deterministic_forward
-    def forward(self, x, features=None):
-        return super().forward(x, features).squeeze(dim=1)
+    def forward(self, x, features=None, rows=None):
+        return super().forward(x, features, rows).squeeze(dim=1)
 
     @staticmethod
     def preprocess(images_u8, net_size=512, net_h=None, resize_mode="minimal", mean=0.5, std=0.5, dtype=None):
@@ -178,9 +194,16 @@
     def infer_batch(self, images_u8, net_size=512, resize_mode="minimal", mean=0.5, std=0.5, net_h=None):
         b, h, w, _ = images_u8.shape
         dtype = self.scratch.layer1_rn.weight.dtype
-        x = self.preprocess(images_u8, net_size, net_h, resize_mode, mean, std, dtype=dtype)
-        if x.is_cuda:
-            x = x.contiguous(memory_format=torch.channels_last)
-        pred = self.forward(x)
+        rows = _patch_rows(self, images_u8, net_size, net_h, resize_mode, mean, std, dtype)
+        if rows is not None:
+            pred = self.forward(None, rows=rows)
+        else:
+            x = self.preprocess(images_u8, net_size, net_h, resize_mode, mean, std, dtype=dtype)
+            if x.is_cuda:
+                x = x.contiguous(memory_format=torch.channels_last)
+            pred = self.forward(x)
+        if vm.DEPTH_TAIL and vm.half_on_gpu(pred):
+            from src import _native
+            return _native.upsample_bicubic_to_f32(pred, (h, w))
         pred = F.interpolate(pred.unsqueeze(1), size=(h, w), mode="bicubic", align_corners=False).squeeze(1)
         return pred.float()
diff --git a/stable-diffusion-webui-depthmap-script_amd/src/_native.py b/stable-diffusion-webui-depthmap-script_amd/src/_native.py
--- a/stable-diffusion-webui-depthmap-script_amd/src/_native.py
+++ b/stable-diffusion-webui-depthmap-script_amd/src/_native.py
@@ -21,6 +21,7 @@
     "ds_dwconv_nhwc", "ds_resize_lanczos", "ds_custom_depth_to_f64", "ds_conv3x3_nhwc_circular", "ds_dpt_head_tail_circular",
     "ds_normalmap_wrap", "ds_normalmap_f64_wrap", "ds_normalmap_gradient_f32_wrap", "ds_normalmap_gradient_f16_wrap", "ds_normalmap_gradient_blur_f32_wrap",
     "ds_bilateral_u16",
+    "ds_preprocess_bicubic_rows", "ds_tokens_fixup", "ds_upsample_bicubic_to_f32", "ds_im2col3x3_s2_nhwc",
 ]
 
 
@@ -80,6 +81,11 @@
             L.ds_dpt_head_tail_circular.argtypes = L.ds_dpt_head_tail.argtypes
             L.ds_preprocess_bicubic.argtypes = [vp, vp, vp, ci, ci, ci, ci, ci, ci, ctypes.POINTER(ctypes.c_float),
                                                 ctypes.POINTER(ctypes.c_float), ci, vp]
+            L.ds_preprocess_bicubic_rows.argtypes = [vp, vp, vp, ci, ci, ci, ci, ci, ci, ctypes.POINTER(ctypes.c_float),
+                                                     ctypes.POINTER(ctypes.c_float), ci, ci, ci, ci, vp]
+            L.ds_tokens_fixup.argtypes = [vp, vp, vp, ci, ci, ci, ci, ci, vp]
+            L.ds_upsample_bicubic_to_f32.argtypes = [vp, vp, vp, ci, ci, ci, ci, ci, ci, vp]
+            L.ds_im2col3x3_s2_nhwc.argtypes = [vp, vp, vp, ci, ci, ci, ci, ci, ci, vp]
             L.ds_reassemble_readout.argtypes = [vp, vp, vp, vp, ci, ci, ci, ci, vp]
             L.ds_bias_act_nhwc.argtypes = [vp, vp, vp, vp, vp, vp, i64, ci, ci, ci, vp]
             L.ds_group_norm_nchw.argtypes = [vp, vp, vp, vp, vp, vp, ci, ci, ci, ci, ctypes.c_float, ci, ci, vp]
@@ -986,6 +992,61 @@
     return out
 
 
+def preprocess_bicubic_rows(images_u8, size_hw, mean, std, patch, n_pad, kpad, flip=True, dtype=None, out=None):
+    torch = require_gpu()
+    assert images_u8.is_cuda and images_u8.dtype == torch.uint8 and images_u8.dim() == 4 and images_u8.shape[3] == 3
+    code = {torch.float16: 1, torch.bfloat16: 2}[dtype]
+    x = images_u8.contiguous()
+    b, h, w, _ = x.shape
+    oh, ow = int(size_hw[0]), int(size_hw[1])
+    if out is None:
+        out = torch.empty((b, int(n_pad), int(kpad)), dtype=dtype, device=x.device)
+    assert out.is_contiguous() and out.dtype == dtype and tuple(out.shape) == (b, int(n_pad), int(kpad)) and out.device == x.device
+    m = (ctypes.c_float * 3)(*[float(v) for v in (mean if hasattr(mean, "__len__") else (mean,) * 3)])
+    s = (ctypes.c_float * 3)(*[float(v) for v in (std if hasattr(std, "__len__") else (std,) * 3)])
+    CALLS["ds_preprocess_bicubic_rows"] += 1
+    _check(lib().ds_preprocess_bicubic_rows(ctx_for(_dev_index(x)), x.data_ptr(), out.data_ptr(), b, h, w, oh, ow, 1 if flip else 0, m, s,
+                                            int(patch), int(n_pad), int(kpad), code, _stream(x)))
+    return out
+
+
+def tokens_fixup(tokens, cls, n_valid):
+    torch = require_gpu()
+    b, n_pad, c = tokens.shape
+    assert tokens.is_cuda and tokens.is_contiguous() and tokens.dtype in (torch.float16, torch.bfloat16) and c % 8 == 0
+    assert cls.is_cuda and cls.dtype == tokens.dtype and cls.is_contiguous() and cls.numel() == c and 1 <= n_valid <= n_pad
+    CALLS["ds_tokens_fixup"] += 1
+    _check(lib().ds_tokens_fixup(ctx_for(_dev_index(tokens)), tokens.data_ptr(), cls.data_ptr(), b, n_pad, int(n_valid), c,
+                                 1 if tokens.dtype == torch.float16 else 2, _stream(tokens)))
+    return tokens
+
+
+def upsample_bicubic_to_f32(pred, size_hw):
+    torch = require_gpu()
+    assert pred.is_cuda and pred.dim() == 3 and pred.dtype in (torch.float16, torch.bfloat16)
+    x = pred.contiguous()
+    b, h, w = x.shape
+    oh, ow = int(size_hw[0]), int(size_hw[1])
+    out = torch.empty((b, oh, ow), dtype=torch.float32, device=x.device)
+    CALLS["ds_upsample_bicubic_to_f32"] += 1
+    _check(lib().ds_upsample_bicubic_to_f32(ctx_for(_dev_index(x)), x.data_ptr(), out.data_ptr(), b, h, w, oh, ow,
+                                            1 if x.dtype == torch.float16 else 2, _stream(x)))
+    return out
+
+
+def im2col3x3_s2(x, circular=False):
+    torch = require_gpu()
+    b, c, h, w = x.shape
+    assert x.is_cuda and x.dtype in (torch.float16, torch.bfloat16) and c % 8 == 0
+    xin = x.contiguous(memory_format=torch.channels_last)
+    ho, wo = (h - 1) // 2 + 1, (w - 1) // 2 + 1
+    rows = torch.empty((b * ho * wo, 9 * c), dtype=x.dtype, device=x.device)
+    CALLS["ds_im2col3x3_s2_nhwc"] += 1
+    _check(lib().ds_im2col3x3_s2_nhwc(ctx_for(_dev_index(x)), xin.data_ptr(), rows.data_ptr(), b, h, w, c, 1 if circular else 0,
+                                      1 if x.dtype == torch.float16 else 2, _stream(x)))
+    return rows
+
+
 def upsample_bilinear(x, size=None, scale_factor=None, align_corners=True):
     torch = require_gpu()
     b, c, ih, iw = x.shape
diff --git a/stable-diffusion-webui-depthmap-script_amd/src/vit_mi355x.py b/stable-diffusion-webui-depthmap-script_amd/src/vit_mi355x.py
--- a/stable-diffusion-webui-depthmap-script_amd/src/vit_mi355x.py
+++ b/stable-diffusion-webui-depthmap-script_amd/src/vit_mi355x.py
@@ -378,6 +378,11 @@
     return x, taps
 
 
+PATCH_ROWS = os.environ.get("DS_PATCH_ROWS", "1") != "0"
+DEPTH_TAIL = os.environ.get("DS_DEPTH_TAIL", "1") != "0"
+IM2COL_HIP = os.environ.get("DS_IM2COL", "1") != "0"
+
+
 def interpolate_bilinear(x, size=None, scale_factor=None, align_corners=True):
     if half_on_gpu(x) and x.shape[1] % 8 == 0:
         from . import _native
@@ -493,6 +498,30 @@
     return y.view(b, gh * gw, conv.out_channels)
 
 
+def patch_rows_ok(conv, dtype, size_hw):
+    if not (PATCH_ROWS and PREPROCESS_HIP and not STOCK[0] and invariant() and LINEAR_HIP == "all" and type(conv) is nn.Conv2d
+            and dtype in (torch.float16, torch.bfloat16) and conv.weight.dtype == dtype):
+        return False
+    k = conv.kernel_size
+    return (k[0] == k[1] and k[0] <= 32 and tuple(conv.stride) == tuple(k) and tuple(conv.padding) == (0, 0) and conv.groups == 1
+            and tuple(conv.dilation) == (1, 1) and conv.out_channels % 256 == 0 and conv.in_channels == 3
+            and size_hw[0] >= k[0] and size_hw[1] >= k[1])
+
+
+def patch_rows_geometry(conv, size_hw, batch):
+    p = conv.kernel_size[0]
+    grid = (size_hw[0] // p, size_hw[1] // p)
+    n_valid = grid[0] * grid[1] + 1
+    return grid, n_valid, pad_len(n_valid, batch), (3 * p * p + 127) // 128 * 128
+
+
+def patch_rows_tokens(conv, cls_token, rows, n_valid):
+    from . import _native
+    b, n_pad, kpad = rows.shape
+    t = _native.linear(rows.view(b * n_pad, kpad), _gemm_weight(conv, rows, kpad), conv.bias).view(b, n_pad, conv.out_channels)
+    return _native.tokens_fixup(t, cls_token.detach().reshape(-1), n_valid)
+
+
 def strided3x3_hip_ok(layer, x):
     if not (invariant() and LINEAR_HIP == "all" and half_on_gpu(x) and x.dim() == 4 and type(layer) is nn.Conv2d):
         return False
@@ -502,14 +531,23 @@
             and layer.in_channels % 128 == 0 and 9 * layer.in_channels <= 16384 and x.shape[1] == layer.in_channels)
 
 
+def strided3x3_rows(x, circular, hip=None):
+    b, c, h, w = x.shape
+    if (IM2COL_HIP if hip is None else hip) and c % 8 == 0:
+        from . import _native
+        return _native.im2col3x3_s2(x, circular)
+    ho, wo = (h - 1) // 2 + 1, (w - 1) // 2 + 1
+    xp = F.pad(x, (1, 1, 1, 1), mode="circular") if circular else F.pad(x, (1, 1, 1, 1))
+    xp = xp.permute(0, 2, 3, 1).contiguous()
+    sb, sh, sw, sc = xp.stride()
+    return xp.as_strided((b, ho, wo, 3, 3, c), (sb, 2 * sh, 2 * sw, sh, sw, sc)).reshape(b * ho * wo, 9 * c)
+
+
 def conv_strided3x3(layer, x):
     from . import _native
     b, c, h, w = x.shape
     ho, wo = (h - 1) // 2 + 1, (w - 1) // 2 + 1
-    xp = F.pad(x, (1, 1, 1, 1), mode="circular") if layer.padding_mode == "circular" else F.pad(x, (1, 1, 1, 1))
-    xp = xp.permute(0, 2, 3, 1).contiguous()
-    sb, sh, sw, sc = xp.stride()
-    rows = xp.as_strided((b, ho, wo, 3, 3, c), (sb, 2 * sh, 2 * sw, sh, sw, sc)).reshape(b * ho * wo, 9 * c)
+    rows = strided3x3_rows(x, layer.padding_mode == "circular")
     y = _native.linear(rows, _gemm_weight(layer, x, 9 * c), layer.bias)
     return y.view(b, ho, wo, layer.out_channels).permute(0, 3, 1, 2)
 PREPROCESS_HIP = os.environ.get("DS_PREPROCESS", "1") != "0"
```

After: 907.9 pairs/s (median of 6 runs). +1.0%, better.
